# CoderWZW/ARLib

Measured on AMD Instinct MI355X. Metric: BPR-train interactions/sec (LightGCN d=64 L=3 + BPR + Adam, B=2048), higher is better.
Workload: dtype f32

## Files before the change

arlib_amd/_lib.py:

```python
import ctypes as C
import os

_HERE = os.path.dirname(os.path.abspath(__file__))
LIB_PATH = os.environ.get('ARLIB_AMD_LIB') or os.path.join(_HERE, 'lib', 'libarlib_amd.so')
ABI_VERSION = 27
_lib = None


class ArlError(RuntimeError):
    pass


class arl_csr(C.Structure):
    _fields_ = [('n_rows', C.c_int64), ('nnz', C.c_int64), ('rowptr', C.c_void_p), ('col', C.c_void_p), ('val', C.c_void_p),
                ('chunk', C.c_int32), ('n_chunks', C.c_int64), ('chunk_row', C.c_void_p), ('chunk_begin', C.c_void_p),
                ('chunk_end', C.c_void_p), ('n_long', C.c_int64), ('long_row', C.c_void_p), ('long_first', C.c_void_p),
                ('long_count', C.c_void_p), ('partial', C.c_void_p), ('row_tasks', C.c_void_p)]


class arl_blocked(C.Structure):
    _fields_ = [('n_waves', C.c_int64), ('rows_per_wave', C.c_int64), ('loads_in_flight', C.c_int64), ('wave_ptr', C.c_void_p), ('wave_rows', C.c_void_p), ('rec_col', C.c_void_p),
                ('rec_val', C.c_void_p), ('n_split', C.c_int64), ('split_row', C.c_void_p), ('split_first', C.c_void_p), ('split_count', C.c_void_p),
                ('partial', C.c_void_p), ('waves_per_group', C.c_int64)]


class arl_tiled(C.Structure):
    _fields_ = [('n_sweeps', C.c_int64), ('n_slots', C.c_int64), ('cap', C.c_int64), ('n_cb', C.c_int64), ('nnz', C.c_int64),
                ('n_groups', C.c_int64), ('bin_rows', C.c_void_p), ('seg_ptr', C.c_void_p), ('e_col', C.c_void_p), ('e_val', C.c_void_p),
                ('e_row', C.c_void_p)]


_vp, _i64, _i32, _f = C.c_void_p, C.c_int64, C.c_int32, C.c_float
_SIGS = {
    'arl_abi_version': (C.c_int, []),
    'arl_mt_seed': (C.c_int, [_vp, _vp, _i64]),
    'arl_sampler_shuffle': (C.c_int, [_vp, _vp, _i64]),
    'arl_mt_sample_range': (C.c_int, [_vp, _i64, _i64, C.c_int32, _vp, _vp]),
    'arl_sampler_next_batch': (C.c_int, [_vp, _vp, _i64, _i64, _i32, _vp, _vp, _i64, _vp, _vp, _vp]),
    'arl_norm_adj_values_f32': (C.c_int, [_i64, _vp, _vp, _vp, _vp, _vp, _vp]),
    'arl_norm_adj_values_coo_f32': (C.c_int, [_i64, _vp, _vp, _vp, _vp, _i64, _vp, _vp, _vp]),
    'arl_norm_vals_coo_f32': (C.c_int, [_vp, _vp, _vp, _i64, _vp, _vp, _vp]),
    'arl_spmm_csr_f32': (C.c_int, [C.POINTER(arl_csr), _vp, _i64, _f, _f, _vp, _vp, _vp]),
    'arl_spmm_csr_layersum_f32': (C.c_int, [C.POINTER(arl_csr), _vp, _i64, _vp, _vp, _vp, _vp]),
    'arl_spmm_csr_adam_f32': (C.c_int, [C.POINTER(arl_csr), _vp, _i64, _f, _f, _vp, _vp, _vp, _vp, _vp, _f, _f, _f, _f, _i64, _vp]),
    'arl_spmm_blocked_f32': (C.c_int, [C.POINTER(arl_blocked), _vp, _i64, _f, _f, _vp, _vp, _vp, _vp]),
    'arl_spmm_csr_rscale_f32': (C.c_int, [C.POINTER(arl_csr), _vp, _i64, _vp, _f, _f, _vp, _vp, _vp]),
    'arl_spmm_blocked_rscale_f32': (C.c_int, [C.POINTER(arl_blocked), _vp, _i64, _vp, _f, _f, _vp, _vp, _vp]),
    'arl_spmm_blocked_layersum_f32': (C.c_int, [C.POINTER(arl_blocked), _vp, _i64, _vp, _vp, _vp, _vp]),
    'arl_spmm_blocked_adam_f32': (C.c_int, [C.POINTER(arl_blocked), _vp, _i64, _f, _f, _vp, _vp, _vp, _vp, _vp, _f, _f, _f, _f, _i64, _vp]),
    'arl_lpt_deal': (C.c_int, [_i64, _vp, _i64, _i64, _vp, _vp]),
    'arl_syn_v1_pairs': (_i64, [_i64, _i64, C.c_double, C.c_uint64, C.c_double, _i64, _i64, _vp, _i64]),
    'arl_graph_digest': (C.c_uint64, [_vp, _i64]),
    'arl_spmm_tiled_f32': (C.c_int, [C.POINTER(arl_tiled), _vp, _i64, _f, _f, _vp, _vp, _vp, _vp]),
    'arl_spmm_tiled_adam_f32': (C.c_int, [C.POINTER(arl_tiled), _vp, _i64, _f, _f, _vp, _vp, _vp, _vp, _vp, _f, _f, _f, _f, _i64, _vp]),
    'arl_spmm_csr_flagged_f32': (C.c_int, [C.POINTER(arl_csr), _vp, _i64, _vp, _f, _f, _vp, _vp, _vp, _vp]),
    'arl_spmm_csr_rows_workspace_bytes': (_i64, [_i64, _i64, _i64]),
    'arl_spmm_csr_rows_f32': (C.c_int, [C.POINTER(arl_csr), _vp, _i64, _vp, _i64, _i64, _vp, _i64, _f, _vp, _vp, _vp, _vp]),
    'arl_mark_rows_u8': (C.c_int, [_vp, _vp, _i64, _i32, _vp]),
    'arl_mark_rows_bits_u32': (C.c_int, [_vp, _vp, _i64, _i32, _vp]),
    'arl_zero_rows_f32': (C.c_int, [_vp, _vp, _i64, _i64, _vp]),
    'arl_batch_rows_set_f32': (C.c_int, [_vp, _vp, _vp, _vp, _i64, _i64, _vp, _f, _vp, _vp, _vp]),
    'arl_batch_rows_clear_f32': (C.c_int, [_vp, _vp, _vp, _vp, _i64, _i64, _vp, _vp]),
    'arl_bpr_l2_workspace_bytes': (_i64, [_i64]),
    'arl_bpr_l2_fwd_bwd_f32': (C.c_int, [_vp, _i64, _i64, _vp, _vp, _vp, _i64, _f, _f, _vp, _vp, _vp, _i32, _vp]),
    'arl_bpr_l2_partial_f32': (C.c_int, [_vp, _i64, _i64, _vp, _vp, _vp, _i64, _i64, _vp, _vp, _vp]),
    'arl_bpr_l2_backward_f32': (C.c_int, [_vp, _i64, _i64, _vp, _vp, _vp, _i64, _f, _f, _vp, _vp, _vp, _vp]),
    'arl_adam_dense_f32': (C.c_int, [_vp, _vp, _vp, _vp, _i64, _f, _f, _f, _f, _i64, _vp]),
    'arl_sgd_dense_f32': (C.c_int, [_vp, _vp, _i64, _f, _vp]),
    'arl_gather_rows_f32': (C.c_int, [_vp, _vp, _i64, _i64, _vp, _vp]),
    'arl_scatter_add_rows_f32': (C.c_int, [_vp, _vp, _i64, _i64, _vp, _f, _vp]),
    'arl_rows_axpy_unique_f32': (C.c_int, [_vp, _vp, _vp, _i64, _i64, _f, _vp, _vp]),
    'arl_shard_batch_prep_i32': (C.c_int, [_vp, _vp, _vp, _i64, _i64, _i64, _vp, _vp, _vp, _vp, _vp]),
    'arl_infonce_workspace_bytes': (_i64, [_i64, _i64]),
    'arl_infonce_fwd_bwd_f32': (C.c_int, [_vp, _vp, _i64, _i64, _f, _f, _vp, _vp, _vp, _vp, _vp]),
    'arl_simgcl_perturb_f32': (C.c_int, [_vp, _vp, _i64, _i64, _f, _vp]),
    'arl_simgcl_perturb_rng_f32': (C.c_int, [_vp, _vp, _i64, _i64, _vp, _f, C.c_uint64, C.c_uint64, _vp]),
    'arl_ngcf_combine_f32': (C.c_int, [_vp, _vp, _i64, _i64, _vp, _vp]),
    'arl_ngcf_act_f32': (C.c_int, [_vp, _vp, _i64, _i64, _f, _vp]),
    'arl_ngcf_act_bwd_f32': (C.c_int, [_vp, _vp, _i64, _i64, _f, _vp, _vp]),
    'arl_ngcf_combine_bwd_f32': (C.c_int, [_vp, _vp, _vp, _i64, _i64, _vp, _vp, _vp]),
    'arl_ngcf_dense_fwd_f32': (C.c_int, [_vp, _vp, _vp, _i64, _i64, _f, _vp, _vp]),
    'arl_ngcf_dense_dgrad_f32': (C.c_int, [_vp, _vp, _vp, _vp, _vp, _i64, _i64, _f, _vp, _vp, _vp, _vp]),
    'arl_ngcf_wgrad_workspace_bytes': (_i64, [_i64, _i64]),
    'arl_ngcf_dense_wgrad_f32': (C.c_int, [_vp, _vp, _vp, _i64, _i64, _vp, _vp, _vp]),
    'arl_ncf_tower_fwd_f32': (C.c_int, [_vp, _vp, _vp, _i64, _i64, _vp, _vp, _vp, _vp, _vp, _vp, _vp, _vp, _vp, _vp]),
    'arl_ncf_tower_bwd_workspace_bytes': (_i64, [_i64, _i64]),
    'arl_ncf_tower_bwd_f32': (C.c_int, [_vp, _vp, _vp, _vp, _vp, _vp, _i64, _i64, _vp, _vp, _vp, _vp, _vp, _vp, _vp]),
    'arl_wrmf_l2_workspace_bytes': (_i64, [_i64]),
    'arl_wrmf_l2_fwd_bwd_f32': (C.c_int, [_vp, _i64, _i64, _vp, _vp, _vp, _i64, _f, _f, _f, _vp, _vp, _vp, _i32, _vp]),
    'arl_sfa_workspace_bytes': (_i64, [_i64, _i64]),
    'arl_sfa_l1_fwd_bwd_f32': (C.c_int, [_vp, _vp, _vp, _i64, _i64, _i64, _f, C.c_int32, _vp, _vp, _vp, _vp]),
    'arl_sfa_stage1_f32': (C.c_int, [_vp, _vp, _vp, _i64, _i64, _vp, _vp, _vp]),
    'arl_sfa_stage2_f32': (C.c_int, [_vp, _vp, _vp, _i64, _i64, _vp, _vp, _vp]),
    'arl_sfa_stage3_f32': (C.c_int, [_vp, _vp, _vp, _vp, _vp, _i64, _i64, _i64, _f, C.c_int32, _vp, _vp, _vp, _vp]),
    'arl_sddmm_csr_f32': (C.c_int, [_vp, _vp, _i64, _i64, _vp, _vp, _f, _vp, _vp]),
    'arl_sddmm_rows_dense_f32': (C.c_int, [_vp, _vp, _i64, _vp, _i64, _i64, _i64, _vp, _vp]),
    'arl_pga_update_f32': (C.c_int, [_vp, _vp, _vp, _vp, _i64, _i64, _vp]),
    'arl_tables_sum_f32': (C.c_int, [_vp, _i64, _i64, C.c_float, _vp, _vp]),
    'arl_fake_block_rows_workspace_bytes': (_i64, [_i64, _i64, _i64]),
    'arl_fake_block_rows_f32': (C.c_int, [_vp, _i64, _i64, _vp, _i64, _vp, C.c_float, _vp, _vp, _vp]),
    'arl_fake_block_cols_f32': (C.c_int, [_vp, _i64, _i64, _vp, _i64, _vp, C.c_float, _vp, _vp]),
    'arl_cw_topk_term_workspace_bytes': (_i64, [_i64, _i64, _i64, _i64]),
    'arl_cw_topk_term_f32': (C.c_int, [_vp, _i64, _i64, _i64, _i64, _vp, _i64, _vp, _i64, C.c_float, _vp, _vp, _vp, _vp, _vp]),
    'arl_score_mask_topk_workspace_bytes': (_i64, [_i64, _i64]),
    'arl_score_mask_topk_stats_offset': (_i64, [_i64, _i64]),
    'arl_score_mask_topk_user_workspace_bytes': (_i64, [_i64, _i64]),
    'arl_score_mask_topk_f32': (C.c_int, [_vp, _vp, _i64, _i64, _i64, _vp, _vp, _i64, _vp, _vp, _vp, _vp, _vp, _vp, C.c_int32, _vp, _vp]),
    'arl_normalize_rows_f32': (C.c_int, [_vp, _i64, _i64, _vp, _vp, _vp]),
    'arl_normalize_rows_bwd_f32': (C.c_int, [_vp, _vp, _vp, _i64, _i64, _f, _vp, _vp, _vp]),
    'arl_nce_allrows_workspace_bytes': (_i64, [_i64, _i64, _i64]),
    'arl_nce_allrows_lse_f32': (C.c_int, [_vp, _i64, _vp, _i64, _i64, _f, _vp, _vp, _vp]),
    'arl_nce_allrows_grad_f32': (C.c_int, [_vp, _i64, _vp, _i64, _i64, _f, _vp, C.c_int32, _vp, _vp, _vp, _vp]),
    'arl_ssl_dropout_nce_workspace_bytes': (_i64, [_i64, _i64]),
    'arl_ssl_dropout_nce_f32': (C.c_int, [_vp, _vp, _i64, _i64, _f, _f, _f, C.c_uint64, C.c_uint64, _vp, _vp, _vp, _vp, _vp, _vp]),
    'arl_gan_gemm_f32': (C.c_int, [_i64, _i64, _i64, _vp, _i64, _i64, _vp, _i64, _i64, _vp, _i32, _vp, _vp, _vp]),
    'arl_gan_spmm_f32': (C.c_int, [_i64, _i64, _vp, _vp, _vp, _vp, _vp, _i32, _vp, _vp]),
    'arl_gan_transpose_f32': (C.c_int, [_vp, _i64, _i64, _vp, _vp]),
    'arl_gan_rows_f32': (C.c_int, [_vp, _vp, _i64, _i64, _i64, _vp, _vp, _vp, _vp, _vp, _vp, _vp]),
    'arl_gan_dz2_f32': (C.c_int, [_vp, _vp, _vp, _vp, _vp, _i64, _i64, _i64, _vp, _vp]),
    'arl_gan_colsum_workspace_bytes': (_i64, [_i64, _i64]),
    'arl_gan_colsum_f32': (C.c_int, [_vp, _vp, _vp, _vp, _i64, _i64, _vp, _vp, _vp]),
    'arl_gan_hash_key': (C.c_uint64, [C.c_uint64, C.c_uint64]),
    'arl_gan_template_i32': (C.c_int, [_i64, _i64, _i64, _vp, _vp, _vp, _vp, _vp, _vp, _vp, _vp, C.c_uint64, C.c_uint64, _vp, _vp, _vp, _vp, _vp]),
    'arl_gan_hash_mask_u8': (C.c_int, [_i64, _i64, _vp, _vp, C.c_uint64, C.c_uint64, _vp, _vp]),
    'arl_gan_threshold_f32': (C.c_int, [_vp, _i64, _i64, _f, _vp, _vp, _vp, _vp]),
    'arl_comm_load': (C.c_int, [C.c_char_p]),
    'arl_comm_unique_id': (C.c_int, [_vp]),
    'arl_comm_init': (C.c_int, [_vp, _i64, _i64, _i64, C.POINTER(C.c_void_p)]),
    'arl_comm_destroy': (C.c_int, [_vp]),
    'arl_item_exchange_range': (C.c_int, [_i64, _i64, _i64, _i64, _i64, C.POINTER(_i64), C.POINTER(_i64)]),
    'arl_allreduce_item_workspace_bytes': (_i64, [_i64, _i64, _i64]),
    'arl_allreduce_item_f32': (C.c_int, [_vp, _vp, _i64, _i64, _vp, _vp]),
    'arl_topn_project_rows_f32': (C.c_int, [_vp, _i64, _i64, _i64, _vp, _vp, _vp, _vp]),
}
EXPORTS = tuple(_SIGS)


def lib():
    global _lib
    if _lib is None:
        if not os.path.exists(LIB_PATH):
            raise ArlError('arlib_amd: %s is missing -- the HIP extension is the product and there is no CPU fallback. '
                           'Build it with `make -C arlib_amd/csrc` (hipcc --offload-arch=gfx950).' % LIB_PATH)
        import torch
        l = C.CDLL(LIB_PATH)
        for name, (res, args) in _SIGS.items():
            fn = getattr(l, name)
            fn.restype, fn.argtypes = res, args
        if l.arl_abi_version() != ABI_VERSION:
            raise ArlError('arlib_amd: ABI version mismatch (lib %d, python %d): rebuild' % (l.arl_abi_version(), ABI_VERSION))
        _lib = l
    return _lib


_ERR = {-1: 'ARL_E_NULL (required pointer is NULL)', -2: 'ARL_E_DIM (unsupported embedding size/shape)',
        -3: 'ARL_E_RANGE (size outside the int32 index range)', -4: 'ARL_E_ARG (inconsistent arguments)'}


def check(rc, what):
    if rc != 0:
        raise ArlError('%s failed: %s' % (what, _ERR.get(rc, 'hipError_t %d' % rc)))
```

arlib_amd/csrc/arl_host.cpp:

```cpp
#include <cstdint>
#include <cstddef>
#include <queue>
#include <cmath>
#include <algorithm>
#include <utility>
#include <vector>
#include "arlib_amd.h"

namespace {

class PyMersenne {
public:
    explicit PyMersenne(uint32_t *state) : w_(state), pos_(state[kN]) {}
    ~PyMersenne() { w_[kN] = pos_; }

    uint32_t next32() {
        if (pos_ >= kN) refill();
        uint32_t y = w_[pos_++];
        y ^= y >> 11;
        y ^= (y << 7) & 0x9d2c5680u;
        y ^= (y << 15) & 0xefc60000u;
        return y ^ (y >> 18);
    }

    uint32_t below(uint32_t n) {
        if (n == 0) return 0;
        const int shift = __builtin_clz(n);
        uint32_t r;
        do { r = next32() >> shift; } while (r >= n);
        return r;
    }

    static void seed_by_array(uint32_t *w, const uint32_t *key, int64_t len) {
        w[0] = 19650218u;
        for (uint32_t i = 1; i < kN; ++i) w[i] = 1812433253u * (w[i - 1] ^ (w[i - 1] >> 30)) + i;
        uint32_t i = 1;
        int64_t j = 0;
        for (int64_t k = (len > (int64_t)kN ? len : (int64_t)kN); k > 0; --k) {
            w[i] = (w[i] ^ ((w[i - 1] ^ (w[i - 1] >> 30)) * 1664525u)) + key[j] + (uint32_t)j;
            if (++i >= kN) { w[0] = w[kN - 1]; i = 1; }
            if (++j >= len) j = 0;
        }
        for (uint32_t k = kN - 1; k > 0; --k) {
            w[i] = (w[i] ^ ((w[i - 1] ^ (w[i - 1] >> 30)) * 1566083941u)) - i;
            if (++i >= kN) { w[0] = w[kN - 1]; i = 1; }
        }
        w[0] = 0x80000000u;
        w[kN] = kN;
    }

private:
    static constexpr uint32_t kN = 624, kM = 397;
    static uint32_t twist(uint32_t hi, uint32_t lo, uint32_t far) {
        const uint32_t y = (hi & 0x80000000u) | (lo & 0x7fffffffu);
        return far ^ (y >> 1) ^ ((y & 1u) ? 0x9908b0dfu : 0u);
    }
    void refill() {
        for (uint32_t k = 0; k < kN - kM; ++k) w_[k] = twist(w_[k], w_[k + 1], w_[k + kM]);
        for (uint32_t k = kN - kM; k < kN - 1; ++k) w_[k] = twist(w_[k], w_[k + 1], w_[k + kM - kN]);
        w_[kN - 1] = twist(w_[kN - 1], w_[0], w_[kM - 1]);
        pos_ = 0;
    }
    uint32_t *w_;
    uint32_t pos_;
};

inline bool user_has_item(const int64_t *rowptr, const int32_t *items, int64_t rows, int32_t user, int32_t item) {
    if (user < 0 || user >= rows) return false;
    const int32_t *lo = items + rowptr[user], *hi = items + rowptr[user + 1];
    while (lo < hi) {
        const int32_t *mid = lo + (hi - lo) / 2;
        if (*mid < item) lo = mid + 1; else hi = mid;
    }
    return lo < items + rowptr[user + 1] && *lo == item;
}

}

extern "C" {

int arl_abi_version(void) { return 27; }

int arl_mt_seed(uint32_t *mt_state, const uint32_t *key, int64_t key_len) {
    if (!mt_state || !key) return ARL_E_NULL;
    if (key_len < 1) return ARL_E_ARG;
    PyMersenne::seed_by_array(mt_state, key, key_len);
    return ARL_OK;
}

int arl_sampler_shuffle(uint32_t *mt_state, int32_t *pairs, int64_t nnz) {
    if (!mt_state || (!pairs && nnz > 0)) return ARL_E_NULL;
    if (nnz < 0 || nnz > 0xFFFFFFFFll) return ARL_E_RANGE;
    if (mt_state[624] > 624) return ARL_E_ARG;
    PyMersenne rng(mt_state);
    int64_t *rows = reinterpret_cast<int64_t *>(pairs);
    const bool aligned = (reinterpret_cast<uintptr_t>(pairs) & 7u) == 0;
    constexpr int kAhead = 512;
    int64_t js[kAhead];
    for (int64_t i = nnz - 1; i >= 1;) {
        const int cnt = (int)(i < kAhead ? i : kAhead);
        for (int t = 0; t < cnt; ++t) {
            js[t] = rng.below((uint32_t)(i - t + 1));
            __builtin_prefetch(pairs + 2 * js[t], 1, 0);
        }
        if (aligned) {
            for (int t = 0; t < cnt; ++t) { const int64_t a = i - t, j = js[t], v = rows[a]; rows[a] = rows[j]; rows[j] = v; }
        } else {
            for (int t = 0; t < cnt; ++t)
                for (int c = 0; c < 2; ++c) { const int64_t a = i - t, j = js[t]; const int32_t v = pairs[2 * a + c]; pairs[2 * a + c] = pairs[2 * j + c]; pairs[2 * j + c] = v; }
        }
        i -= cnt;
    }
    return ARL_OK;
}

int arl_mt_sample_range(uint32_t *mt_state, int64_t n, int64_t k, int32_t use_pool, int32_t *out, int32_t *scratch) {
    if (!mt_state || (!out && k > 0) || !scratch) return ARL_E_NULL;
    if (n < 0 || k < 0 || k > n || n > 0x7FFFFFFFll) return ARL_E_ARG;
    if (mt_state[624] > 624) return ARL_E_ARG;
    PyMersenne rng(mt_state);
    if (use_pool) {
        for (int64_t i = 0; i < n; ++i) scratch[i] = (int32_t)i;
        for (int64_t i = 0; i < k; ++i) {
            const uint32_t j = rng.below((uint32_t)(n - i));
            out[i] = scratch[j];
            scratch[j] = scratch[n - i - 1];
        }
    } else {
        uint32_t *seen = reinterpret_cast<uint32_t *>(scratch);
        for (int64_t w = 0; w < (n + 31) / 32; ++w) seen[w] = 0u;
        for (int64_t i = 0; i < k; ++i) {
            uint32_t j = rng.below((uint32_t)n);
            while ((seen[j >> 5] >> (j & 31)) & 1u) j = rng.below((uint32_t)n);
            seen[j >> 5] |= 1u << (j & 31);
            out[i] = (int32_t)j;
        }
    }
    return ARL_OK;
}

int arl_sampler_next_batch(uint32_t *mt_state, const int32_t *pairs, int64_t begin, int64_t count, int32_t n_items,
                           const int64_t *memb_rowptr, const int32_t *memb_items, int64_t memb_rows,
                           int32_t *out_u, int32_t *out_p, int32_t *out_n) {
    if (!mt_state || !pairs || !out_u || !out_p || !out_n) return ARL_E_NULL;
    if (memb_rows > 0 && (!memb_rowptr || !memb_items)) return ARL_E_NULL;
    if (begin < 0 || count < 0 || n_items <= 0) return ARL_E_ARG;
    if (mt_state[624] > 624) return ARL_E_ARG;
    PyMersenne rng(mt_state);
    for (int64_t b = 0; b < count; ++b) {
        const int32_t user = pairs[2 * (begin + b)], pos = pairs[2 * (begin + b) + 1];
        int32_t neg;
        do { neg = (int32_t)rng.below((uint32_t)n_items); }
        while (user_has_item(memb_rowptr, memb_items, memb_rows, user, neg));
        out_u[b] = user; out_p[b] = pos; out_n[b] = neg;
    }
    return ARL_OK;
}

int arl_lpt_deal(int64_t n, const int32_t *weight_desc, int64_t n_bins, int64_t cap, int32_t *bin_out, int32_t *slot_out) {
    if (n < 0 || n_bins < 0 || cap < 1 || n_bins > 0x7fffffffll || n_bins * cap < n) return ARL_E_ARG;
    if (n == 0) return ARL_OK;
    if (!weight_desc || !bin_out || !slot_out) return ARL_E_NULL;
    typedef std::pair<int64_t, int32_t> Load;
    std::priority_queue<Load, std::vector<Load>, std::greater<Load>> open;
    std::vector<int32_t> fill((size_t)n_bins, 0);
    for (int64_t b = 0; b < n_bins; ++b) open.push(Load(0, (int32_t)b));
    for (int64_t r = 0; r < n; ++r) {
        if (weight_desc[r] < 0 || (r > 0 && weight_desc[r] > weight_desc[r - 1])) return ARL_E_ARG;
        const Load top = open.top();
        open.pop();
        bin_out[r] = top.second;
        slot_out[r] = fill[top.second]++;
        if (fill[top.second] < cap) open.push(Load(top.first + weight_desc[r], top.second));
    }
    return ARL_OK;
}

static inline uint64_t syn_splitmix64(uint64_t x) {
    x += 0x9E3779B97F4A7C15ull;
    uint64_t z = x;
    z = (z ^ (z >> 30)) * 0xBF58476D1CE4E5B9ull;
    z = (z ^ (z >> 27)) * 0x94D049BB133111EBull;
    return z ^ (z >> 31);
}
static inline uint64_t syn_hash(uint64_t base, uint64_t index) { return syn_splitmix64(index ^ base); }
static inline uint64_t syn_base(uint64_t seed, uint64_t stream) { return syn_splitmix64(seed ^ (stream * 0x9E3779B97F4A7C15ull)); }
static inline double syn_uniform(uint64_t h) { return ((double)(h >> 11) + 0.5) * (1.0 / 9007199254740992.0); }

int64_t arl_syn_v1_pairs(int64_t n_users, int64_t n_items, double mean_deg, uint64_t seed, double sigma, int64_t deg_min, int64_t deg_max,
                         int32_t *pairs_out, int64_t capacity) {
    if (n_users <= 0 || n_items <= 0 || n_users > 0x7fffffffll || n_items > 0x7fffffffll || !(mean_deg > 0) || !(sigma >= 0) || deg_min < 0 || deg_max < deg_min)
        return ARL_E_ARG;
    const uint64_t b1 = syn_base(seed, 1), b2 = syn_base(seed, 2), b3 = syn_base(seed, 3), b4 = syn_base(seed, 4), b5 = syn_base(seed, 5);
    const double mu = std::log(mean_deg) - 0.5 * sigma * sigma;
    const double two_pi = 2.0 * 3.14159265358979323846;
    const int64_t hi = deg_max < n_items ? deg_max : n_items;
    std::vector<int64_t> deg((size_t)n_users);
    int64_t total = 0;
    for (int64_t u = 0; u < n_users; ++u) {
        const double u1 = syn_uniform(syn_hash(b1, (uint64_t)u)), u2 = syn_uniform(syn_hash(b2, (uint64_t)u));
        const double z = std::sqrt(-2.0 * std::log(u1)) * std::cos(two_pi * u2);
        double dg = std::nearbyint(std::exp(mu + sigma * z));
        if (dg < (double)deg_min) dg = (double)deg_min;
        if (dg > (double)hi) dg = (double)hi;
        deg[(size_t)u] = (int64_t)dg;
        total += deg[(size_t)u];
    }
    std::vector<std::pair<uint64_t, int64_t>> hp((size_t)n_items);
    for (int64_t j = 0; j < n_items; ++j) hp[(size_t)j] = std::make_pair(syn_hash(b4, (uint64_t)j), j);
    std::stable_sort(hp.begin(), hp.end(), [](const std::pair<uint64_t, int64_t> &a, const std::pair<uint64_t, int64_t> &b) { return a.first < b.first; });
    std::vector<int64_t> keys;
    keys.reserve((size_t)(total + n_items));
    int64_t k = 0;
    for (int64_t u = 0; u < n_users; ++u)
        for (int64_t t = 0; t < deg[(size_t)u]; ++t, ++k) {
            const double r = syn_uniform(syn_hash(b3, (uint64_t)k));
            int64_t pos = (int64_t)((double)n_items * r * r);
            if (pos > n_items - 1) pos = n_items - 1;
            keys.push_back(u * n_items + hp[(size_t)pos].second);
        }
    for (int64_t j = 0; j < n_items; ++j) keys.push_back((int64_t)(syn_hash(b5, (uint64_t)j) % (uint64_t)n_users) * n_items + j);
    std::sort(keys.begin(), keys.end());
    keys.erase(std::unique(keys.begin(), keys.end()), keys.end());
    const int64_t nnz = (int64_t)keys.size();
    if (!pairs_out || capacity < nnz) return nnz;
    for (int64_t e = 0; e < nnz; ++e) {
        pairs_out[2 * e] = (int32_t)(keys[(size_t)e] / n_items);
        pairs_out[2 * e + 1] = (int32_t)(keys[(size_t)e] % n_items);
    }
    return nnz;
}

uint64_t arl_graph_digest(const int32_t *pairs, int64_t n) {
    uint64_t acc = 0;
// ... 10 lines not shown
```

arlib_amd/csrc/arl_kernels.hip:

```cpp
#include <hip/hip_runtime.h>
#include <stdint.h>
#include <math.h>
#include <stdio.h>
#include <stdlib.h>
#include "arlib_amd.h"
#include <type_traits>

#define ARL_LAUNCH_CHECK()                                  \
    do {                                                    \
        hipError_t e__ = hipGetLastError();                 \
        if (e__ != hipSuccess) return (int)e__;             \
    } while (0)

namespace {

constexpr int kWave = 64;
constexpr int kBlock = 256;
constexpr int kWavesPerBlock = kBlock / kWave;

__device__ __forceinline__ float wave_sum(float v) {
#pragma unroll
    for (int off = 32; off > 0; off >>= 1) v += __shfl_xor(v, off);
    return v;
}
// ... 97 lines not shown
            y.x = fmaf(ep.beta, z.x, y.x); y.y = fmaf(ep.beta, z.y, y.y); y.z = fmaf(ep.beta, z.z, y.z); y.w = fmaf(ep.beta, z.w, y.w);
        }
        *reinterpret_cast<float4 *>(ep.Y + o) = y;
    } else if (MODE == EPI_LAYERSUM) {
        const float4 s = *reinterpret_cast<const float4 *>(ep.S_in + o);
        if (ep.Y) *reinterpret_cast<float4 *>(ep.Y + o) = a;
        *reinterpret_cast<float4 *>(ep.S + o) = add4(s, a);
    } else {
        float g[4] = {ep.alpha * a.x, ep.alpha * a.y, ep.alpha * a.z, ep.alpha * a.w};
        if (ep.Z && (!ep.zflags || ep.zflags[row])) {
            const float4 z = *reinterpret_cast<const float4 *>(ep.Z + o);
            g[0] = fmaf(ep.beta, z.x, g[0]); g[1] = fmaf(ep.beta, z.y, g[1]); g[2] = fmaf(ep.beta, z.z, g[2]); g[3] = fmaf(ep.beta, z.w, g[3]);
        }
        float4 p4 = *reinterpret_cast<const float4 *>(ep.P + o);
        float4 m4 = *reinterpret_cast<const float4 *>(ep.M + o);
        float4 v4 = *reinterpret_cast<const float4 *>(ep.V + o);
        float p[4] = {p4.x, p4.y, p4.z, p4.w}, m[4] = {m4.x, m4.y, m4.z, m4.w}, v[4] = {v4.x, v4.y, v4.z, v4.w};
#pragma unroll
        for (int k = 0; k < 4; ++k) {
            m[k] = m[k] + (g[k] - m[k]) * ep.w1;
            v[k] = v[k] * ep.b2 + ep.w2 * g[k] * g[k];
            const float denom = sqrtf(v[k]) / ep.bc2_sqrt + ep.eps;
            p[k] = p[k] - ep.step_size * (m[k] / denom);
        }
        *reinterpret_cast<float4 *>(ep.P + o) = make_float4(p[0], p[1], p[2], p[3]);
        *reinterpret_cast<float4 *>(ep.M + o) = make_float4(m[0], m[1], m[2], m[3]);
        *reinterpret_cast<float4 *>(ep.V + o) = make_float4(v[0], v[1], v[2], v[3]);
    }
}

template <int LPR, int MODE>
__global__ __launch_bounds__(kBlock) void spmm_rows_kernel(CsrDev A, const float *__restrict__ X, int d, Epi ep) {
    const int lane = threadIdx.x & (kWave - 1);
    const long long task = (long long)blockIdx.x * kWavesPerBlock + (threadIdx.x >> 6);
    const int q = lane % LPR;
    if (task < A.n_chunks) {
        const int t = (int)task;
        float4 a = spmm_gather<LPR, 4>(A.col, A.val, A.chunk_begin[t], A.chunk_end[t], X, d, lane);
        a = group_reduce<LPR>(a);
        if (lane < LPR && q * 4 < d) *reinterpret_cast<float4 *>(A.partial + (size_t)t * d + q * 4) = a;
        return;
    }
    const long long r = task - A.n_chunks;
    if (r >= A.n_rows) return;
    const int begin = A.rowptr[r], end = A.rowptr[r + 1];
    if (A.n_chunks > 0 && end - begin > A.chunk) return;
    float4 a = spmm_gather<LPR, 4>(A.col, A.val, begin, end, X, d, lane);
    a = group_reduce<LPR>(a);
    if (lane < LPR && q * 4 < d) spmm_epilogue<MODE>(ep, (int)r, d, q, a);
}

template <int LPR, int MODE>
__global__ __launch_bounds__(kBlock) void spmm_long_rows_kernel(CsrDev A, int d, Epi ep) {
    constexpr int G = kWave / LPR;
    const int lane = threadIdx.x & (kWave - 1);
    const int t = blockIdx.x * kWavesPerBlock + (threadIdx.x >> 6);
    if (t >= A.n_long) return;
    const int g = lane / LPR, q = lane % LPR;
    const int first = A.long_first[t], cnt = A.long_count[t];
    float4 a = make_float4(0.f, 0.f, 0.f, 0.f);
    if (q * 4 < d)
        for (int s = g; s < cnt; s += G) a = add4(a, *reinterpret_cast<const float4 *>(A.partial + (size_t)(first + s) * d + q * 4));
    a = group_reduce<LPR>(a);
    if (lane < LPR && q * 4 < d) spmm_epilogue<MODE>(ep, A.long_row[t], ep.ld ? ep.ld : d, q, a);
}


template <int LPR, int MODE>
__global__ __launch_bounds__(kBlock) void spmm_rows_masked_gpr_kernel(CsrDev A, const float *__restrict__ X, int d, Epi ep,
                                                                        const uint32_t *__restrict__ xbits) {
    constexpr int G = kWave / LPR;
    const int lane = threadIdx.x & (kWave - 1);
    const int g = lane / LPR, q = lane % LPR;
    const long long task = ((long long)blockIdx.x * kWavesPerBlock + (threadIdx.x >> 6)) * G + g;
    const long long total = (long long)A.n_chunks + A.n_rows;
    int begin = 0, end = 0, row = -1, slot = -1;
    if (task < A.n_chunks) {
        slot = (int)task; begin = A.chunk_begin[slot]; end = A.chunk_end[slot];
    } else if (task < total) {
        if (A.row_tasks) {
            const int4 rt = A.row_tasks[task - A.n_chunks];
            row = rt.x; begin = rt.y; end = rt.z;
        } else {
            row = (int)(task - A.n_chunks);
            begin = A.rowptr[row]; end = A.rowptr[row + 1];
        }
        if (A.n_chunks > 0 && end - begin > A.chunk) { end = begin; row = -1; }
    }
    const bool qact = (q * 4 < d);
    const float *xq = X + q * 4;
    float4 acc = make_float4(0.f, 0.f, 0.f, 0.f);
    for (int base = begin; __any(base < end); base += 2 * LPR) {
        const int e0 = base + q, e1 = base + LPR + q;
        int c0 = 0, c1 = 0;
        if (e0 < end) c0 = A.col[e0];
        if (e1 < end) c1 = A.col[e1];
        bool f0 = false, f1 = false;
        if (e0 < end) f0 = (xbits[c0 >> 5] >> (c0 & 31)) & 1u;
        if (e1 < end) f1 = (xbits[c1 >> 5] >> (c1 & 31)) & 1u;
        const unsigned long long wm0 = __ballot(f0), wm1 = __ballot(f1);
#pragma unroll
        for (int half = 0; half < 2; ++half) {
            const unsigned long long wm = half ? wm1 : wm0;
            const int c = half ? c1 : c0;
            unsigned long long mask = (wm >> (g * LPR)) & ((LPR == 64) ? ~0ull : ((1ull << (LPR & 63)) - 1ull));
            while (mask) {
                const int j = __ffsll((long long)mask) - 1;
                mask &= mask - 1ull;
                const int cj = __shfl(c, g * LPR + j);
                const float vj = A.val[base + half * LPR + j];
                if (qact) fma4(acc, vj, *reinterpret_cast<const float4 *>(xq + (size_t)cj * d));
            }
        }
    }
    if (!qact) return;
    if (slot >= 0) *reinterpret_cast<float4 *>(A.partial + (size_t)slot * d + q * 4) = acc;
    else if (row >= 0) spmm_epilogue<MODE>(ep, row, d, q, acc);
}

struct LayerPtrs { const float *p[8]; int n; };

template <int LPR>
__global__ __launch_bounds__(kBlock) void spmm_subset_kernel(CsrDev A, const float *__restrict__ X, int d, const int32_t *__restrict__ rows, int n,
                                                              int nsplit, float *__restrict__ partial) {
    const int lane = threadIdx.x & (kWave - 1);
    const long long task = (long long)blockIdx.x * kWavesPerBlock + (threadIdx.x >> 6);
    if (task >= (long long)n * nsplit) return;
    const int t = (int)(task / nsplit), sp = (int)(task % nsplit);
    const int r = rows[t];
    const int begin = A.rowptr[r], end = A.rowptr[r + 1];
    const int per = (end - begin + nsplit - 1) / nsplit;
    const int b = begin + sp * per, e = min(end, b + per);
    const int q = lane % LPR;
    float4 a = make_float4(0.f, 0.f, 0.f, 0.f);
    if (b < e) a = spmm_gather<LPR, 4>(A.col, A.val, b, e, X, d, lane);
    a = group_reduce<LPR>(a);
    if (lane < LPR && q * 4 < d) *reinterpret_cast<float4 *>(partial + (size_t)task * d + q * 4) = a;
}

template <int LPR>
__global__ __launch_bounds__(kBlock) void subset_finish_kernel(const float *__restrict__ partial, int n, int nsplit, int d, const int32_t *__restrict__ rows,
                                                                LayerPtrs L, float alpha, float *__restrict__ out_c, const float *__restrict__ row_weight) {
    constexpr int G = kWave / LPR;
    const int lane = threadIdx.x & (kWave - 1);
    const int g = lane / LPR, q = lane % LPR;
    const int t = (blockIdx.x * kWavesPerBlock + (threadIdx.x >> 6)) * G + g;
    if (t >= n || q * 4 >= d) return;
    const int r = rows[t];
    float4 a = make_float4(0.f, 0.f, 0.f, 0.f);
    for (int k = 0; k < L.n; ++k) a = add4(a, *reinterpret_cast<const float4 *>(L.p[k] + (size_t)r * d + q * 4));
    for (int s = 0; s < nsplit; ++s) a = add4(a, *reinterpret_cast<const float4 *>(partial + ((size_t)t * nsplit + s) * d + q * 4));
    const float w = row_weight ? alpha * row_weight[t] : alpha;
    *reinterpret_cast<float4 *>(out_c + (size_t)t * d + q * 4) = make_float4(w * a.x, w * a.y, w * a.z, w * a.w);
}

__global__ __launch_bounds__(kBlock) void tables_sum_kernel(LayerPtrs L, long long n4, float alpha, float4 *__restrict__ out) {
    for (long long t = (long long)blockIdx.x * kBlock + threadIdx.x; t < n4; t += (long long)gridDim.x * kBlock) {
        float4 a = reinterpret_cast<const float4 *>(L.p[0])[t];
        for (int k = 1; k < L.n; ++k) a = add4(a, reinterpret_cast<const float4 *>(L.p[k])[t]);
        out[t] = make_float4(alpha * a.x, alpha * a.y, alpha * a.z, alpha * a.w);
    }
}

__global__ __launch_bounds__(kBlock) void mark_rows_kernel(uint8_t *__restrict__ flags, const int32_t *__restrict__ idx, int n, int value) {
    const int t = blockIdx.x * kBlock + threadIdx.x;
    if (t < n) flags[idx[t]] = (uint8_t)value;
}
__global__ __launch_bounds__(kBlock) void mark_bits_kernel(uint32_t *__restrict__ bits, const int32_t *__restrict__ idx, int n, int set) {
    const int t = blockIdx.x * kBlock + threadIdx.x;
    if (t >= n) return;
    const int i = idx[t];
    if (set) atomicOr(bits + (i >> 5), 1u << (i & 31));
    else atomicAnd(bits + (i >> 5), ~(1u << (i & 31)));
}
__global__ __launch_bounds__(kBlock) void zero_rows_kernel(float *__restrict__ dst, const int32_t *__restrict__ idx, int n, int d) {
    const int lane = threadIdx.x & 63;
    const int t = blockIdx.x * kWavesPerBlock + (threadIdx.x >> 6);
    if (t >= n) return;
    float *o = dst + (size_t)idx[t] * d;
    for (int k = lane; k < d; k += kWave) o[k] = 0.f;
}

constexpr int kOrderedWindow = 16384;

template <class RowOf, class OnHit>
__device__ __forceinline__ bool ordered_scan(int c0, int c1, int t, long long row, int lane, RowOf rowof, OnHit on_hit) {
    for (int base = c0; base < c1; base += 256) {
        long long v[4];
#pragma unroll
        for (int i = 0; i < 4; ++i) {
            const int j = base + 64 * i + lane;
            v[i] = j < c1 ? (long long)rowof(j) : -1ll;
        }
#pragma unroll
        for (int i = 0; i < 4; ++i) {
            unsigned long long m = __ballot(v[i] == row);
            const int b0 = base + 64 * i;
            if (b0 < t) {
                const int lim = t - b0;
                if (lim >= 64 ? m != 0ull : (m & ((1ull << lim) - 1ull)) != 0ull) return false;
            }
            while (m) {
                const int tt = b0 + __ffsll((long long)m) - 1;
                m &= m - 1ull;
                on_hit(tt);
            }
        }
    }
    return true;
}

template <class OnHit>
__device__ __forceinline__ bool ordered_scan_lds(const int32_t *srows, int c0, int c1, int t, int row, int lane, OnHit on_hit) {
    const int n = c1 - c0, tl = t - c0;
    for (int base = 0; base < n; base += 512) {
        int v[8];
#pragma unroll
        for (int i = 0; i < 8; ++i) {
            const int j = base + 64 * i + lane;
            v[i] = j < n ? srows[j] : -1;
        }
#pragma unroll
        for (int i = 0; i < 8; ++i) {
            unsigned long long m = __ballot(v[i] == row);
            const int b0 = base + 64 * i;
            if (b0 < tl) {
                const int lim = tl - b0;
                if (lim >= 64 ? m != 0ull : (m & ((1ull << lim) - 1ull)) != 0ull) return false;
            }
            while (m) {
                const int tt = c0 + b0 + __ffsll((long long)m) - 1;
                m &= m - 1ull;
                on_hit(tt);
            }
        }
    }
    return true;
}
template <class OnGroup>
__device__ __forceinline__ bool ordered_scan_lds_groups(const int32_t *srows, int c0, int c1, int t, int row, int lane, OnGroup on_group) {
    const int n = c1 - c0, tl = t - c0;
    for (int base = 0; base < n; base += 512) {
        int v[8];
#pragma unroll
        for (int i = 0; i < 8; ++i) {
            const int j = base + 64 * i + lane;
            v[i] = j < n ? srows[j] : -1;
        }
#pragma unroll
        for (int i = 0; i < 8; ++i) {
            const unsigned long long m = __ballot(v[i] == row);
            const int b0 = base + 64 * i;
            if (b0 < tl) {
                const int lim = tl - b0;
                if (lim >= 64 ? m != 0ull : (m & ((1ull << lim) - 1ull)) != 0ull) return false;
            }
            if (m) on_group(m, c0 + b0);
        }
    }
    return true;
}
template <class RowOf>
__device__ __forceinline__ void stage_rows(int32_t *srows, int c0, int c1, RowOf rowof) {
    for (int j = threadIdx.x; j < c1 - c0; j += kBlock) srows[j] = (int32_t)rowof(c0 + j);
    __syncthreads();
}

__global__ __launch_bounds__(kBlock) void rows_mark_dups_kernel(uint32_t *__restrict__ bits, uint32_t *__restrict__ dup, const int32_t *__restrict__ idx, int n,
                                                                 const float *__restrict__ row_scale) {
    const int t = blockIdx.x * kBlock + threadIdx.x;
    if (t >= n) return;
    if (row_scale && row_scale[t] == 0.f) return;
    const int row = idx[t];
    const uint32_t m = 1u << (row & 31);
    if (atomicOr(bits + (row >> 5), m) & m) atomicOr(dup + (row >> 5), m);
}

template <bool MARK>
__global__ __launch_bounds__(kBlock) void rows_add_ordered_kernel(float *__restrict__ dst, uint8_t *__restrict__ flags, uint32_t *__restrict__ bits,
                                                                   const int32_t *__restrict__ idx, int c0, int c1, int d,
                                                                   const float *__restrict__ src, float scale, const float *__restrict__ row_scale,
                                                                   const uint32_t *__restrict__ dup) {
    extern __shared__ int32_t srows[];
    const int lane = threadIdx.x & 63;
    const int t = c0 + blockIdx.x * kWavesPerBlock + (threadIdx.x >> 6);
    const bool valid = t < c1 && !(row_scale && row_scale[t] == 0.f);
    const int row = valid ? idx[t] : 0;
    float *o = dst + (size_t)row * d;
    const bool fast = valid && dup && !((dup[row >> 5] >> (row & 31)) & 1u);
    if (fast) {
        const float sc = row_scale ? scale * row_scale[t] : scale;
        const float *s = src + (size_t)t * d;
        for (int k = lane; k < d; k += kWave) {
#pragma clang fp contract(off)
            const float c = sc * s[k];
            o[k] = o[k] + c;
        }
        if (MARK && lane == 0) flags[row] = 1;
    }
    if (!__syncthreads_or(valid && !fast)) return;
    stage_rows(srows, c0, c1, [&](int j) { return (row_scale && row_scale[j] == 0.f) ? -1 : idx[j]; });
    if (!valid || fast) return;
    for (int k0 = 0; k0 < d; k0 += 256) {
        float acc[4];
#pragma unroll
        for (int i = 0; i < 4; ++i) { const int k = k0 + 64 * i + lane; acc[i] = k < d ? o[k] : 0.f; }
// ... 3633 lines not shown
    if (beta != 0.f && !Z) return ARL_E_NULL;
    if (Y == X) return ARL_E_ARG;
    Epi ep = {};
    ep.alpha = alpha; ep.beta = beta; ep.Z = (beta != 0.f) ? Z : nullptr; ep.Y = Y;
    return launch_spmm<EPI_AXPBY>(A, X, d, ep, (hipStream_t)stream);
}

int arl_spmm_csr_rscale_f32(const arl_csr *A, const float *X, int64_t d, const float *row_scale, float alpha, float beta, const float *Z, float *Y,
                            arl_stream_t stream) {
    if (!Y || !row_scale) return ARL_E_NULL;
    if (beta != 0.f && !Z) return ARL_E_NULL;
    if (Y == X) return ARL_E_ARG;
    Epi ep = {};
    ep.alpha = alpha; ep.beta = beta; ep.Z = (beta != 0.f) ? Z : nullptr; ep.Y = Y; ep.rscale = row_scale;
    return launch_spmm<EPI_AXPBY>(A, X, d, ep, (hipStream_t)stream);
}

int arl_spmm_csr_layersum_f32(const arl_csr *A, const float *X, int64_t d, const float *S_in, float *S, float *Y, arl_stream_t stream) {
    if (!S_in || !S) return ARL_E_NULL;
    if (Y == X) return ARL_E_ARG;
    Epi ep = {};
    ep.S_in = S_in; ep.S = S; ep.Y = Y;
    return launch_spmm<EPI_LAYERSUM>(A, X, d, ep, (hipStream_t)stream);
}

int arl_spmm_blocked_f32(const arl_blocked *P, const float *X, int64_t d, float alpha, float beta, const float *Z, const uint8_t *zflags, float *Y,
                         arl_stream_t stream) {
    if (!Y) return ARL_E_NULL;
    if (beta != 0.f && !Z) return ARL_E_NULL;
    if (Y == X) return ARL_E_ARG;
    Epi ep = {};
    ep.alpha = alpha; ep.beta = beta; ep.Z = (beta != 0.f) ? Z : nullptr; ep.zflags = zflags; ep.Y = Y;
    return launch_spmm_blocked<EPI_AXPBY>(P, X, d, ep, (hipStream_t)stream);
}

int arl_spmm_blocked_rscale_f32(const arl_blocked *P, const float *X, int64_t d, const float *row_scale, float alpha, float beta, const float *Z,
                                float *Y, arl_stream_t stream) {
    if (!Y || !row_scale) return ARL_E_NULL;
    if (beta != 0.f && !Z) return ARL_E_NULL;
    if (Y == X) return ARL_E_ARG;
    Epi ep = {};
    ep.alpha = alpha; ep.beta = beta; ep.Z = (beta != 0.f) ? Z : nullptr; ep.Y = Y; ep.rscale = row_scale;
    return launch_spmm_blocked<EPI_AXPBY>(P, X, d, ep, (hipStream_t)stream);
}

int arl_spmm_blocked_layersum_f32(const arl_blocked *P, const float *X, int64_t d, const float *S_in, float *S, float *Y, arl_stream_t stream) {
    if (!S_in || !S) return ARL_E_NULL;
    if (Y == X) return ARL_E_ARG;
    Epi ep = {};
    ep.S_in = S_in; ep.S = S; ep.Y = Y;
    return launch_spmm_blocked<EPI_LAYERSUM>(P, X, d, ep, (hipStream_t)stream);
}

int arl_spmm_blocked_adam_f32(const arl_blocked *P, const float *X, int64_t d, float alpha, float beta, const float *Z, const uint8_t *zflags,
                              float *Pm, float *M, float *V, float lr, float beta1, float beta2, float eps, int64_t step, arl_stream_t stream) {
    if (!Pm || !M || !V) return ARL_E_NULL;
    if (beta != 0.f && !Z) return ARL_E_NULL;
    if (step < 1 || Pm == X) return ARL_E_ARG;
    Epi ep = {};
    ep.alpha = alpha; ep.beta = beta; ep.Z = (beta != 0.f) ? Z : nullptr; ep.zflags = zflags; ep.P = Pm; ep.M = M; ep.V = V;
    {
        const AdamScalars a = adam_scalars(lr, beta1, beta2, step);
        ep.step_size = a.step_size; ep.bc2_sqrt = a.bc2_sqrt; ep.w1 = a.w1; ep.b2 = a.b2; ep.w2 = a.w2; ep.eps = (float)typed_double(eps);
    }
    return launch_spmm_blocked<EPI_ADAM>(P, X, d, ep, (hipStream_t)stream);
}

int arl_spmm_tiled_f32(const arl_tiled *T, const float *X, int64_t d, float alpha, float beta, const float *Z, const uint8_t *zflags, float *Y,
                       arl_stream_t stream) {
    if (!Y) return ARL_E_NULL;
    if (beta != 0.f && !Z) return ARL_E_NULL;
    if (Y == X) return ARL_E_ARG;
    Epi ep = {};
    ep.alpha = alpha; ep.beta = beta; ep.Z = (beta != 0.f) ? Z : nullptr; ep.zflags = zflags; ep.Y = Y;
    return launch_spmm_tiled<EPI_AXPBY>(T, X, d, ep, (hipStream_t)stream);
}

int arl_spmm_tiled_adam_f32(const arl_tiled *T, const float *X, int64_t d, float alpha, float beta, const float *Z, const uint8_t *zflags,
                            float *P, float *M, float *V, float lr, float beta1, float beta2, float eps, int64_t step, arl_stream_t stream) {
    if (!P || !M || !V) return ARL_E_NULL;
    if (beta != 0.f && !Z) return ARL_E_NULL;
    if (step < 1 || P == X) return ARL_E_ARG;
    Epi ep = {};
    ep.alpha = alpha; ep.beta = beta; ep.Z = (beta != 0.f) ? Z : nullptr; ep.zflags = zflags; ep.P = P; ep.M = M; ep.V = V;
    {
        const AdamScalars a = adam_scalars(lr, beta1, beta2, step);
        ep.step_size = a.step_size; ep.bc2_sqrt = a.bc2_sqrt; ep.w1 = a.w1; ep.b2 = a.b2; ep.w2 = a.w2; ep.eps = (float)typed_double(eps);
    }
    return launch_spmm_tiled<EPI_ADAM>(T, X, d, ep, (hipStream_t)stream);
}

int arl_spmm_csr_flagged_f32(const arl_csr *A, const float *X, int64_t d, const uint32_t *xbits, float alpha, float beta, const float *Z,
                             const uint8_t *zflags, float *Y, arl_stream_t stream) {
    if (!Y) return ARL_E_NULL;
    if (beta != 0.f && !Z) return ARL_E_NULL;
    if (Y == X) return ARL_E_ARG;
    Epi ep = {};
    ep.alpha = alpha; ep.beta = beta; ep.Z = (beta != 0.f) ? Z : nullptr; ep.zflags = zflags; ep.Y = Y;
    return launch_spmm<EPI_AXPBY>(A, X, d, ep, (hipStream_t)stream, xbits);
}

int arl_spmm_csr_adam_f32(const arl_csr *A, const float *X, int64_t d, float alpha, float beta, const float *Z, const uint8_t *zflags, float *P,
                          float *M, float *V, float lr, float beta1, float beta2, float eps, int64_t step, arl_stream_t stream) {
    if (!P || !M || !V) return ARL_E_NULL;
    if (beta != 0.f && !Z) return ARL_E_NULL;
    if (step < 1) return ARL_E_ARG;
    if (P == X) return ARL_E_ARG;
    Epi ep = {};
    ep.alpha = alpha; ep.beta = beta; ep.Z = (beta != 0.f) ? Z : nullptr; ep.zflags = zflags; ep.P = P; ep.M = M; ep.V = V;
    {
        const AdamScalars a = adam_scalars(lr, beta1, beta2, step);
        ep.step_size = a.step_size; ep.bc2_sqrt = a.bc2_sqrt; ep.w1 = a.w1; ep.b2 = a.b2; ep.w2 = a.w2; ep.eps = (float)typed_double(eps);
    }
    return launch_spmm<EPI_ADAM>(A, X, d, ep, (hipStream_t)stream);
}

int64_t arl_spmm_csr_rows_workspace_bytes(int64_t n_rows_sel, int64_t nsplit, int64_t d) {
    return (n_rows_sel < 0 || nsplit < 1 || d < 0) ? 0 : (int64_t)sizeof(float) * n_rows_sel * nsplit * d;
}

int arl_spmm_csr_rows_f32(const arl_csr *A, const float *X, int64_t d, const int32_t *rows, int64_t n_rows_sel, int64_t nsplit,
                          const float *const *layers, int64_t n_layers, float alpha, const float *row_weight, float *out_c, void *workspace,
                          arl_stream_t stream) {
    if (!A || !X || !rows || !out_c || !workspace || !A->rowptr) return ARL_E_NULL;
    if (A->nnz > 0 && (!A->col || !A->val)) return ARL_E_NULL;
    if (n_layers < 0 || n_layers > 8 || (n_layers > 0 && !layers)) return ARL_E_ARG;
    if (d <= 0 || d > 256 || (d & 3)) return ARL_E_DIM;
    if (n_rows_sel < 0 || nsplit < 1 || nsplit > 1024 || n_rows_sel * nsplit > 0x7fffffffll) return ARL_E_RANGE;
    if (n_rows_sel == 0) return ARL_OK;
    hipStream_t st = (hipStream_t)stream;
    CsrDev D = {};
    D.n_rows = (int)A->n_rows; D.rowptr = A->rowptr; D.col = A->col; D.val = A->val;
    LayerPtrs LP = {};
    LP.n = (int)n_layers;
    for (int k = 0; k < LP.n; ++k) { if (!layers[k]) return ARL_E_NULL; LP.p[k] = layers[k]; }
    const long long tasks = n_rows_sel * nsplit;
    const unsigned grid = (unsigned)((tasks + kWavesPerBlock - 1) / kWavesPerBlock);
    const int di = (int)d, n = (int)n_rows_sel, ns = (int)nsplit;
    float *part = (float *)workspace;
#define ARL_SUBSET_CASE(LPRV)                                                                                                  \
    do {                                                                                                                       \
        hipLaunchKernelGGL((spmm_subset_kernel<LPRV>), dim3(grid), dim3(kBlock), 0, st, D, X, di, rows, n, ns, part);          \
        ARL_LAUNCH_CHECK();                                                                                                    \
        const unsigned g2 = (unsigned)((n + kWavesPerBlock * (kWave / LPRV) - 1) / (kWavesPerBlock * (kWave / LPRV)));         \
        hipLaunchKernelGGL((subset_finish_kernel<LPRV>), dim3(g2), dim3(kBlock), 0, st, part, n, ns, di, rows, LP, alpha, out_c, row_weight); \
        ARL_LAUNCH_CHECK();                                                                                                    \
    } while (0)
    if (d <= 16) ARL_SUBSET_CASE(4);
    else if (d <= 32) ARL_SUBSET_CASE(8);
    else if (d <= 64) ARL_SUBSET_CASE(16);
    else if (d <= 128) ARL_SUBSET_CASE(32);
    else ARL_SUBSET_CASE(64);
#undef ARL_SUBSET_CASE
    return ARL_OK;
}

int arl_mark_rows_u8(uint8_t *flags, const int32_t *idx, int64_t n, int32_t value, arl_stream_t stream) {
    if (!flags || !idx) return ARL_E_NULL;
    if (n < 0 || n > 0x7fffffffll) return ARL_E_ARG;
    if (n == 0) return ARL_OK;
    hipLaunchKernelGGL(mark_rows_kernel, dim3((unsigned)((n + kBlock - 1) / kBlock)), dim3(kBlock), 0, (hipStream_t)stream, flags, idx, (int)n, (int)value);
    ARL_LAUNCH_CHECK();
    return ARL_OK;
}

int arl_mark_rows_bits_u32(uint32_t *bits, const int32_t *idx, int64_t n, int32_t set, arl_stream_t stream) {
    if (!bits || !idx) return ARL_E_NULL;
    if (n < 0 || n > 0x7fffffffll) return ARL_E_ARG;
    if (n == 0) return ARL_OK;
    hipLaunchKernelGGL(mark_bits_kernel, dim3((unsigned)((n + kBlock - 1) / kBlock)), dim3(kBlock), 0, (hipStream_t)stream, bits, idx, (int)n, (int)set);
    ARL_LAUNCH_CHECK();
    return ARL_OK;
}

int arl_batch_rows_set_f32(float *G, uint8_t *flags, uint32_t *bits, const int32_t *idx, int64_t n, int64_t d, const float *src, float scale,
                           const float *row_scale, uint32_t *dup_bits, arl_stream_t stream) {
    if (!G || !flags || !bits || !idx || !src) return ARL_E_NULL;
    if (n < 0 || n > 0x7fffffffll || d <= 0 || d > 0x7fffffffll) return ARL_E_ARG;
    if (n == 0) return ARL_OK;
    if (dup_bits) {
        hipLaunchKernelGGL(rows_mark_dups_kernel, dim3((unsigned)((n + kBlock - 1) / kBlock)), dim3(kBlock), 0, (hipStream_t)stream, bits, dup_bits, idx, (int)n, row_scale);
        ARL_LAUNCH_CHECK();
    }
    for (int64_t c0 = 0; c0 < n; c0 += kOrderedWindow) {
        const int64_t c1 = c0 + kOrderedWindow < n ? c0 + kOrderedWindow : n;
        hipLaunchKernelGGL(rows_add_ordered_kernel<true>, dim3((unsigned)((c1 - c0 + kWavesPerBlock - 1) / kWavesPerBlock)), dim3(kBlock), (size_t)(c1 - c0) * 4,
                           (hipStream_t)stream, G, flags, bits, idx, (int)c0, (int)c1, (int)d, src, scale, row_scale, (const uint32_t *)dup_bits);
        ARL_LAUNCH_CHECK();
    }
    return ARL_OK;
}

int arl_batch_rows_clear_f32(float *G, uint8_t *flags, uint32_t *bits, const int32_t *idx, int64_t n, int64_t d, uint32_t *dup_bits, arl_stream_t stream) {
    if (!G || !flags || !bits || !idx) return ARL_E_NULL;
    if (n < 0 || n > 0x7fffffffll || d <= 0 || d > 0x7fffffffll) return ARL_E_ARG;
    if (n == 0) return ARL_OK;
    hipLaunchKernelGGL(batch_rows_clear_kernel, dim3((unsigned)((n + kWavesPerBlock - 1) / kWavesPerBlock)), dim3(kBlock), 0, (hipStream_t)stream, G, flags,
                       bits, idx, (int)n, (int)d, dup_bits);
    ARL_LAUNCH_CHECK();
    return ARL_OK;
}

int arl_zero_rows_f32(float *dst, const int32_t *idx, int64_t n, int64_t d, arl_stream_t stream) {
    if (!dst || !idx) return ARL_E_NULL;
    if (n < 0 || d <= 0 || n > 0x7fffffffll || d > 0x7fffffffll) return ARL_E_ARG;
    if (n == 0) return ARL_OK;
    hipLaunchKernelGGL(zero_rows_kernel, dim3((unsigned)((n + kWavesPerBlock - 1) / kWavesPerBlock)), dim3(kBlock), 0, (hipStream_t)stream, dst, idx, (int)n, (int)d);
    ARL_LAUNCH_CHECK();
    return ARL_OK;
}

int64_t arl_bpr_l2_workspace_bytes(int64_t B) { return B < 0 ? 0 : (int64_t)sizeof(float) * 4 * B; }

int arl_bpr_l2_fwd_bwd_f32(const float *emb, int64_t d, int64_t item_off, const int32_t *u, const int32_t *p, const int32_t *n, int64_t B,
                           float reg, float upstream, float *loss_out, float *G, void *workspace, int32_t distinct_rows, arl_stream_t stream) {
    if (!emb || !u || !p || !n || !loss_out || !workspace) return ARL_E_NULL;
    if (d <= 0 || B <= 0 || item_off < 0) return ARL_E_ARG;
    if (B > 0x7fffffffll / 4 || d > 0x7fffffffll) return ARL_E_RANGE;
    hipStream_t st = (hipStream_t)stream;
    float *ws = (float *)workspace;
    const unsigned grid = (unsigned)((B + kWavesPerBlock - 1) / kWavesPerBlock);
    hipLaunchKernelGGL(bpr_fwd_kernel, dim3(grid), dim3(kBlock), 0, st, emb, (int)d, (long long)item_off, u, p, n, (int)B, (float)B, ws);
    ARL_LAUNCH_CHECK();
    hipLaunchKernelGGL(bpr_finalize_kernel, dim3(1), dim3(kBlock), 0, st, (int)B, reg, ws, loss_out, 0);
    ARL_LAUNCH_CHECK();
    if (G) {
        const int rc = launch_bpr_bwd(emb, d, item_off, u, p, n, B, reg, upstream, ws, loss_out, G, st, distinct_rows != 0);
        if (rc) return rc;
    }
    return ARL_OK;
}

int arl_bpr_l2_partial_f32(const float *emb, int64_t d, int64_t item_off, const int32_t *u, const int32_t *p, const int32_t *n, int64_t B_local,
                           int64_t B_global, float *sums_out, void *workspace, arl_stream_t stream) {
    if (!emb || !sums_out || !workspace) return ARL_E_NULL;
    if (B_local > 0 && (!u || !p || !n)) return ARL_E_NULL;
    if (d <= 0 || B_local < 0 || B_global < B_local || B_global <= 0 || item_off < 0) return ARL_E_ARG;
    if (B_local > 0x7fffffffll / 4 || d > 0x7fffffffll) return ARL_E_RANGE;
    hipStream_t st = (hipStream_t)stream;
    float *ws = (float *)workspace;
    if (B_local > 0) {
        const unsigned grid = (unsigned)((B_local + kWavesPerBlock - 1) / kWavesPerBlock);
        hipLaunchKernelGGL(bpr_fwd_kernel, dim3(grid), dim3(kBlock), 0, st, emb, (int)d, (long long)item_off, u, p, n, (int)B_local, (float)B_global, ws);
        ARL_LAUNCH_CHECK();
    }
    hipLaunchKernelGGL(bpr_finalize_kernel, dim3(1), dim3(kBlock), 0, st, (int)B_local, 0.f, ws, sums_out, 1);
    ARL_LAUNCH_CHECK();
    return ARL_OK;
}

int arl_bpr_l2_backward_f32(const float *emb, int64_t d, int64_t item_off, const int32_t *u, const int32_t *p, const int32_t *n, int64_t B_local,
                            float reg, float upstream, const float *norms4, float *G, const void *workspace, arl_stream_t stream) {
    if (!emb || !norms4 || !G || !workspace) return ARL_E_NULL;
    if (B_local > 0 && (!u || !p || !n)) return ARL_E_NULL;
    if (d <= 0 || B_local < 0 || item_off < 0) return ARL_E_ARG;
    if (B_local > 0x7fffffffll / 4 || d > 0x7fffffffll) return ARL_E_RANGE;
    if (B_local == 0) return ARL_OK;
    return launch_bpr_bwd(emb, d, item_off, u, p, n, B_local, reg, upstream, (const float *)workspace, norms4, G, (hipStream_t)stream);
}

int arl_adam_dense_f32(float *p, const float *g, float *m, float *v, int64_t n, float lr, float beta1, float beta2, float eps, int64_t step,
                       arl_stream_t stream) {
    if (!p || !g || !m || !v) return ARL_E_NULL;
    if (n < 0 || step < 1) return ARL_E_ARG;
    if (n == 0) return ARL_OK;
    const AdamScalars a = adam_scalars(lr, beta1, beta2, step);
    hipStream_t st = (hipStream_t)stream;
    const bool al = (((uintptr_t)p | (uintptr_t)g | (uintptr_t)m | (uintptr_t)v) & 15u) == 0;
    const long long n4 = al ? n / 4 : 0;
    if (n4 > 0) {
        hipLaunchKernelGGL(adam_kernel, dim3(grid_for(n4, kBlock)), dim3(kBlock), 0, st, (float4 *)p, (const float4 *)g, (float4 *)m, (float4 *)v, n4,
                           a.step_size, a.bc2_sqrt, a.w1, a.b2, a.w2, eps);
        ARL_LAUNCH_CHECK();
    }
    if (n4 * 4 < n) {
        hipLaunchKernelGGL(adam_scalar_kernel, dim3(grid_for(n - n4 * 4, kBlock)), dim3(kBlock), 0, st, p, g, m, v, n4 * 4, (long long)n, a.step_size,
                           a.bc2_sqrt, a.w1, a.b2, a.w2, eps);
        ARL_LAUNCH_CHECK();
    }
    return ARL_OK;
}

int arl_sgd_dense_f32(float *p, const float *g, int64_t n, float lr, arl_stream_t stream) {
    if (!p || !g) return ARL_E_NULL;
    if (n < 0) return ARL_E_ARG;
    if (n == 0) return ARL_OK;
    hipLaunchKernelGGL(sgd_kernel, dim3(grid_for(n, kBlock)), dim3(kBlock), 0, (hipStream_t)stream, p, g, (long long)n, lr);
    ARL_LAUNCH_CHECK();
    return ARL_OK;
}

int arl_tables_sum_f32(const float *const *tables, int64_t n_tables, int64_t n_elems, float alpha, float *out, arl_stream_t stream) {
    if (!tables || !out) return ARL_E_NULL;
    if (n_tables < 1 || n_tables > 8 || n_elems < 0 || (n_elems & 3)) return ARL_E_ARG;
    if (n_elems == 0) return ARL_OK;
    LayerPtrs LP = {};
    LP.n = (int)n_tables;
    for (int k = 0; k < LP.n; ++k) { if (!tables[k]) return ARL_E_NULL; LP.p[k] = tables[k]; }
    const long long n4 = n_elems / 4;
    hipLaunchKernelGGL(tables_sum_kernel, dim3(grid_for(n4, kBlock)), dim3(kBlock), 0, (hipStream_t)stream, LP, n4, alpha, (float4 *)out);
    ARL_LAUNCH_CHECK();
    return ARL_OK;
}

int arl_gather_rows_f32(const float *src, const int32_t *idx, int64_t n, int64_t d, float *dst, arl_stream_t stream) {
    if (!src || !idx || !dst) return ARL_E_NULL;
// ... 912 lines not shown
```

arlib_amd/engine.py:

```python
import torch

from . import ops


def mean_adjacency_gradient(A, E0, G, L, s, out, noises=None, eps=0.1):
    if L == 0:
        return out
    E = [E0]
    for k in range(L - 1):
        nxt = ops.spmm(A, E[-1])
        if noises is not None:
            ops.simgcl_perturb_(nxt, noises[k], eps)
        E.append(nxt)
    G = G.contiguous()
    acc = G
    for j in range(L):
        ops.sddmm_csr(A, acc, E[L - 1 - j], s, out=out)
        if j < L - 1:
            acc = ops.spmm(A, acc, 1.0, 1.0, G)
    return out


class PropagationEngine:
    def __init__(self, graph, n_users, n_items, emb_size, n_layers, reg, lr, device, skip_layer0=False,
                 optimizer='adam', betas=(0.9, 0.999), eps=1e-8, table=None, schedule='auto'):
        self.A = graph
        self.U, self.I, self.d, self.L = int(n_users), int(n_items), int(emb_size), int(n_layers)
        self.N = self.U + self.I
        self.reg, self.lr, self.betas, self.eps = float(reg), float(lr), betas, eps
        self.skip0 = bool(skip_layer0)
        self.optimizer = optimizer
        self.device = torch.device(device)
        if self.device.type != 'cuda':
            raise ops._lib.ArlError('PropagationEngine needs a GPU device (no CPU fallback)')
        if graph is None and self.L > 0:
            raise ValueError('n_layers > 0 needs a graph')
        if graph is not None and graph.n_rows != self.N:
            raise ValueError('graph has %d rows, expected U+I=%d' % (graph.n_rows, self.N))
        if self.L > 0:
            ops._check_width(self.d, 'PropagationEngine')
        if self.skip0 and self.L < 1:
            raise ValueError('skip_layer0 needs n_layers >= 1')
        if schedule not in ('auto', 'csr', 'blocked'):
            raise ValueError("schedule must be 'auto', 'csr' or 'blocked'")
        if schedule != 'csr':
            ops.auto_blocked(graph, emb_size, split=self.U, force=(schedule == 'blocked'))
        if graph is not None and graph.nnz >= ops.BLOCKED_MIN_NNZ:
            graph.enable_masked_order()
        z = lambda: torch.zeros(self.N, self.d, dtype=torch.float32, device=self.device)
        self.E0 = z() if table is None else table
        if self.E0.shape != (self.N, self.d) or self.E0.dtype != torch.float32 or not self.E0.is_contiguous():
            raise ValueError('table must be contiguous fp32 [U+I, d]')
        self.m, self.v, self.G = z(), z(), z()
        if self.L > 0:
            self.S, self.Ea, self.Eb = z(), z(), z()
        else:
            self.S = self.E0
        self.t = 0
        self.loss_out = torch.zeros(4, dtype=torch.float32, device=self.device)
        self._G_dirty = True
        self._noise_seed, self._noise_stream = None, 0
        self.nsplit = 32
        self.flags = self.bits = self.dup_bits = self.hops = None
        self._sparse_B, self._sb_cache = None, {}
        self.Gc = self.out_c = self.rows_ws = self.ar = self.arB = self._ws = None
        self._sgl_acc = self._sgl_hops = None
        self.ngcf_W = self.ngcf_m = self.ngcf_v = None

    @property
    def user_emb(self):
        return self.E0[:self.U]

    @property
    def item_emb(self):
        return self.E0[self.U:]

    def forward(self, noises=None, eps=0.1, out=None):
        L, A = self.L, self.A
        if L == 0:
            return self.E0
        S = self.S if out is None else out
        if noises is None and not self.skip0:
            if L == 1:
                return ops.spmm(A, self.E0, 0.5, 0.5, self.E0, out=S)
            ops.spmm_layersum(A, self.E0, self.E0, S, self.Ea)
            cur, nxt = self.Ea, self.Eb
            for _ in range(L - 2):
                ops.spmm_layersum(A, cur, S, S, nxt)
                cur, nxt = nxt, cur
            s = 1.0 / (L + 1)
            return ops.spmm(A, cur, s, s, S, out=S)
        cur, nxt, x = self.Ea, self.Eb, self.E0
        for k in range(L):
            ops.spmm(A, x, out=cur)
            if noises is not None:
                ops.simgcl_perturb_(cur, noises[k], eps)
            if k == 0:
                if self.skip0:
                    S.copy_(cur)
                else:
                    torch.add(self.E0, cur, out=S)
            else:
                S.add_(cur)
            x, cur, nxt = cur, nxt, cur
        S.mul_(1.0 / (L if self.skip0 else L + 1))
        return S

    def backward_to_table(self, G, out=None):
        L, A = self.L, self.A
        if L == 0:
            return G
        acc, dst = self._dense_hops(G)
        if self.skip0:
            return ops.spmm(A, acc, 1.0 / L, out=dst)
        s = 1.0 / (L + 1)
        return ops.spmm(A, acc, s, s, G, out=dst)

    def _dense_hops(self, G):
        acc, bufs = G, (self.Ea, self.Eb)
        for k in range(self.L - 1):
            acc = ops.spmm(self.A, acc, 1.0, 1.0, G, out=bufs[k % 2])
        return acc, bufs[(self.L - 1) % 2]

    def adjacency_gradient(self, G, out=None, noises=None, eps=0.1):
        L, A = self.L, self.A
        if out is None:
            out = torch.zeros(A.col.numel(), dtype=torch.float32, device=G.device)
        return mean_adjacency_gradient(A, self.E0, G, L, 1.0 / L if self.skip0 else 1.0 / (L + 1), out, noises, eps)

    def forward_rows(self, rows):
        L, A = self.L, self.A
        if L == 0 or self.skip0 or L > 8:
            raise ValueError('forward_rows: LightGCN mean over layers 0..L with 1 <= L <= 8')
        n = rows.numel()
        self._sparse_buffers(max(n // 3, 1) if n % 3 == 0 else n)
        return self._mean_rows(A, self.hops, rows)

    def backward_rows(self, rows, g_rows):
        L, A = self.L, self.A
        s = 1.0 / (L + 1)
        self._begin_sparse(self._sparse_B)
        self._set_rows(rows, g_rows.contiguous())
        acc, bits = self._masked_hops(A, self.hops)
        out = ops.spmm_flagged(A, acc, bits, s, s, self.G, self.flags)
        self._clear_rows(rows)
        return out

    def _begin_sparse(self, B):
        self._sparse_buffers(B)
        if self._G_dirty:
            self.G.zero_()
            self._G_dirty = False

    def _batch_rows(self, u, p, n):
        return torch.cat([u, p + self.U, n + self.U])

    def _contrast_rows(self, u, p):
        uidx = torch.unique(u.long())
        iidx = torch.unique(p.long()) + self.U
        return torch.cat([uidx, iidx]).to(torch.int32), uidx.numel()

    def _streams(self, n):
        if self._noise_seed is None:
            self._noise_seed = int(torch.randint(0, 2 ** 62, (1,)).item())
            self._noise_stream = 0
        first = self._noise_stream
        self._noise_stream += n
        return self._noise_seed, first

    def _mean_rows(self, graph, hops, rows, out=None, workspace=None):
        layers = [self.E0]
        for k in range(self.L - 1):
            layers.append(ops.spmm(graph, layers[-1], out=hops[k]))
        return ops.spmm_rows(graph, layers[-1], rows, layers, 1.0 / (self.L + 1), nsplit=self.nsplit, out=out, workspace=workspace, check_range=False)

    def _bpr_compact(self, out_c, B):
        self.Gc.zero_()
        ops.bpr_l2_fwd_bwd(out_c, B, self.ar, self.ar, self.arB, self.reg, self.Gc, workspace=self._ws, loss_out=self.loss_out, check_range=False, distinct_rows=True)

    def _set_rows(self, rows, grad):
        ops.batch_rows_set_(self.G, self.flags, self.bits, rows, grad, 1.0, check_range=False, dup_bits=self.dup_bits)

    def _mark_rows(self, rows):
        ops.mark_rows_(self.flags, rows, 1, check_range=False)
        ops.mark_bits_(self.bits, rows, True, self.N, check_range=False)

    def _clear_rows(self, rows):
        ops.batch_rows_clear_(self.G, self.flags, self.bits, rows, check_range=False, dup_bits=self.dup_bits)

    def _masked_hops(self, graph, bufs, src=None, after_hop=None):
        acc, bits = self.G if src is None else src, self.bits
        for k in range(self.L - 1):
            acc = ops.spmm_flagged(graph, acc, bits, 1.0, 1.0, self.G, self.flags, out=bufs[k % len(bufs)])
            bits = None
            if after_hop is not None:
                after_hop(self.L - 1 - k, acc)
        return acc, bits

    def loss_and_grad_out(self, out, u, p, n):
        self.G.zero_()
        self._G_dirty = True
        if self._ws is None or self._ws.numel() < 4 * u.numel():
            self._ws = torch.empty(4 * u.numel(), dtype=torch.float32, device=self.device)
        ops.bpr_l2_fwd_bwd(out, self.U, u, p, n, self.reg, self.G, workspace=self._ws, loss_out=self.loss_out, check_range=False)
        return self.loss_out

    def grad(self, u, p, n):
        out = self.forward()
        lo = self.loss_and_grad_out(out, u, p, n)
        return lo, self.backward_to_table(self.G)

    def step(self, u, p, n, rows=None):
        if self.optimizer != 'adam' or self.L == 0 or self.skip0 or self.L > 8:
            return self.step_dense(u, p, n)
        return self._step_sparse(u, p, n, rows, None)

    def _step_sparse(self, u, p, n, rows, extra_grad):
        L, A = self.L, self.A
        B = u.numel()
        if rows is None:
            rows = self._batch_rows(u, p, n)
        self._begin_sparse(B)
        s = 1.0 / (L + 1)
        self._mean_rows(A, self.hops, rows, out=self.out_c, workspace=self.rows_ws)
        self._bpr_compact(self.out_c, B)
        if extra_grad is not None:
            extra_grad()
        self._set_rows(rows, self.Gc)
        self.t += 1
        acc, bits = self._masked_hops(A, self.hops)
        if L == 1:
            ops.spmm_flagged(A, acc, bits, s, s, self.G, self.flags, out=self.hops[0])
            ops.adam_dense(self.E0, self.hops[0], self.m, self.v, self.lr, self.t, self.betas, self.eps)
        else:
            ops.spmm_adam(A, acc, s, s, self.G, self.E0, self.m, self.v, self.lr, self.t, self.betas, self.eps, zflags=self.flags)
        self._clear_rows(rows)
        return self.loss_out

    def step_ssl4rec(self, u, p, n, cl_rate=1.0, tau=0.2, drop=0.2, masks=None, seed=None, stream_id=None):
        L, A = self.L, self.A
        if self.optimizer != 'adam' or self.skip0 or L < 1 or L > 8:
            raise ValueError('step_ssl4rec needs a LightGCN-mean engine (no skip_layer0, 1 <= L <= 8) with Adam')
        B = u.numel()
        if self.d not in ops.SSL_NCE_WIDTHS:
            raise ValueError('step_ssl4rec: embedding size %d unsupported (d in %s)' % (self.d, ops.SSL_NCE_WIDTHS))
        if masks is not None and tuple(masks.shape) != (2, 2, B, self.d):
            raise ValueError('step_ssl4rec: masks [2, 2, B, d]')
        if seed is None:
            seed, stream_id = self._streams(1)
        cl = []
        def contrastive():
            loss, _ = ops.ssl_dropout_nce(self.out_c[:B], self.out_c[B:2 * B], drop, tau, G=(self.Gc[:B], self.Gc[B:2 * B]), upstream=cl_rate,
                                          seed=seed, stream_id=stream_id, masks=masks)
            cl.append(loss)
        self._step_sparse(u, p, n, None, contrastive)
        cl = cl[0]
        return self.loss_out, cl_rate * (cl[1] + cl[0])

    def init_ngcf(self, weights):
        if len(weights) != self.L or any(tuple(w.shape) != (self.d, self.d) for pair in weights for w in pair):
            raise ValueError('init_ngcf: one pair of [d, d] weights per layer')
        self.ngcf_W = [(a.data if hasattr(a, 'data') else a, b.data if hasattr(b, 'data') else b) for a, b in weights]
        z = lambda: torch.zeros(self.d, self.d, dtype=torch.float32, device=self.device)
        self.ngcf_m = [(z(), z()) for _ in weights]
        self.ngcf_v = [(z(), z()) for _ in weights]

    def step_ngcf(self, u, p, n, rows=None, slope=0.01, capture=None):
        L, A, d = self.L, self.A, self.d
        if L < 1 or self.ngcf_W is None or d not in ops.NGCF_DENSE_WIDTHS:
            raise ValueError('step_ngcf: needs n_layers >= 1, init_ngcf() and d in %s' % (ops.NGCF_DENSE_WIDTHS,))
        B = u.numel()
        if rows is None:
            rows = self._batch_rows(u, p, n)
        self._begin_sparse(B)
        s = 1.0 / (L + 1)
        Wcat = [torch.cat([a, b], 0) for a, b in self.ngcf_W]
        egos, Ps = [self.E0], []
        for l in range(L - 1):
            P = ops.spmm(A, egos[-1])
            Ps.append(P)
            egos.append(ops.ngcf_dense_fwd(P, egos[-1], Wcat[l], slope))
        P_r = ops.spmm_rows(A, egos[-1], rows, (), 1.0, nsplit=ops.ROWS_NSPLIT, check_range=False)
        E_r = ops.gather_rows(egos[-1], rows, check_range=False)
        out_r = ops.ngcf_dense_fwd(P_r, E_r, Wcat[L - 1], slope)
        acc = out_r + E_r
        for e in egos[:-1]:
            acc += ops.gather_rows(e, rows, check_range=False)
        acc *= s
        self._bpr_compact(acc, B)
        Gs = self.Gc * s
        self.t += 1
        gP_r, gE_r, gW = ops.ngcf_dense_bwd(Gs, out_r, P_r, E_r, Wcat[L - 1], slope)
        gWs = [None] * L
        gWs[L - 1] = gW
        self._set_rows(rows, gP_r)
        g = ops.spmm_flagged(A, self.G, self.bits)
        self._clear_rows(rows)
        ops.scatter_add_rows(g, rows, gE_r + Gs, 1.0, check_range=False)
        if L == 1:
            if capture is not None:
                capture['table'] = g.clone()
            ops.adam_dense(self.E0, g, self.m, self.v, self.lr, self.t, self.betas, self.eps)
        for l in range(L - 2, -1, -1):
            gP, gE, gWs[l] = ops.ngcf_dense_bwd(g, egos[l + 1], Ps[l], egos[l], Wcat[l], slope)
            ops.scatter_add_rows(gE, rows, Gs, 1.0, check_range=False)
            if l > 0:
                g = ops.spmm(A, gP, 1.0, 1.0, gE)
            elif capture is not None:
                capture['table'] = ops.spmm(A, gP, 1.0, 1.0, gE)
                ops.adam_dense(self.E0, capture['table'], self.m, self.v, self.lr, self.t, self.betas, self.eps)
            else:
                ops.spmm_adam(A, gP, 1.0, 1.0, gE, self.E0, self.m, self.v, self.lr, self.t, self.betas, self.eps)
        if capture is not None:
            capture['W'] = [w.clone() for w in gWs]
        for l in range(L):
            for k in range(2):
                ops.adam_dense(self.ngcf_W[l][k], gWs[l][k * d:(k + 1) * d], self.ngcf_m[l][k], self.ngcf_v[l][k], self.lr, self.t, self.betas, self.eps)
        return self.loss_out

    def step_simgcl(self, u, p, n, cl_rate=0.2, tau=0.2, eps=0.1, noises=None):
        if not self.skip0 or self.optimizer != 'adam':
            raise ValueError('step_simgcl needs a skip_layer0 engine with Adam')
        L, A = self.L, self.A
        B = u.numel()
        self._begin_sparse(B)
        inv = 1.0 / L
        rows = self._batch_rows(u, p, n)
        rows_cl, nu = self._contrast_rows(u, p)
        rng_mode = noises is None
        if rng_mode:
            seed, stream0 = self._streams(2 * L)
        rnd = (lambda v, k: noises[v][k]) if noises is not None else None
        def perturb_full(src, v, k, out=None):
            if rng_mode:
                return ops.simgcl_perturb_rng(src, eps, seed, stream0 + v * L + k, out=out)
            dst = src.clone() if out is None else out.copy_(src)
            return ops.simgcl_perturb_(dst, rnd(v, k), eps)
        def perturb_rows(src, v, k, sel):
            if rng_mode:
                return ops.simgcl_perturb_rng(src, eps, seed, stream0 + v * L + k, out=src, row_ids=sel)
            return ops.simgcl_perturb_(src, rnd(v, k)[sel.long()].contiguous(), eps)
        E1 = ops.spmm(A, self.E0, out=self.hops[0])
        def finish(first, view):
            sel = rows if view is None else rows_cl
            layers, cur = [first], first
            for k in range(1, L - 1):
                nxt = ops.spmm(A, cur)
                if view is not None:
                    perturb_full(nxt, view, k, out=nxt)
                layers.append(nxt); cur = nxt
            if L == 1:
                return ops.gather_rows(first, sel, check_range=False)
            if view is None:
                return ops.spmm_rows(A, cur, sel, layers, inv, nsplit=self.nsplit, check_range=False)
            last = ops.spmm_rows(A, cur, sel, (), 1.0, nsplit=self.nsplit, check_range=False)
            perturb_rows(last, view, L - 1, sel)
            for t in layers:
                last += ops.gather_rows(t, sel, check_range=False)
            return last * inv
        out_c = finish(E1, None)
        self._bpr_compact(out_c, B)
        ops.scatter_add_rows(self.G, rows, self.Gc, 1.0, check_range=False)
        views = []
        for v in (0, 1):
            E1p = perturb_full(E1, v, 0)
            views.append(finish(E1p, v))
        lu, du1, du2 = ops.infonce_fwd_bwd(views[0][:nu].contiguous(), views[1][:nu].contiguous(), tau)
        li, di1, di2 = ops.infonce_fwd_bwd(views[0][nu:].contiguous(), views[1][nu:].contiguous(), tau)
        cl_loss = cl_rate * (lu[0] + li[0])
        gcl = torch.cat([du1 + du2, di1 + di2], 0)
        ops.scatter_add_rows(self.G, rows_cl, gcl, cl_rate, check_range=False)
        allrows = torch.cat([rows, rows_cl])
        self._mark_rows(allrows)
        self.t += 1
        acc, bits = self._masked_hops(A, (self.hops[1], self.hops[0]))
        if L == 1:
            tmp = ops.spmm_flagged(A, acc, bits, inv, 0.0, None, None, out=self.hops[1])
            ops.adam_dense(self.E0, tmp, self.m, self.v, self.lr, self.t, self.betas, self.eps)
        else:
            ops.spmm_adam(A, acc, inv, 0.0, None, self.E0, self.m, self.v, self.lr, self.t, self.betas, self.eps)
        self._clear_rows(allrows)
        return self.loss_out, cl_loss

    def step_xsimgcl(self, u, p, n, cl_rate=0.2, tau=0.1, eps=0.1, layer_cl=1, noises=None):
        if not self.skip0 or self.optimizer != 'adam':
            raise ValueError('step_xsimgcl needs a skip_layer0 engine with Adam')
        L, A = self.L, self.A
        if not (1 <= layer_cl <= L):
            raise ValueError('layer_cl must be in [1, L]')
        B = u.numel()
        self._begin_sparse(B)
        inv = 1.0 / L
        rows = self._batch_rows(u, p, n)
        rows_cl, nu = self._contrast_rows(u, p)
        sel = torch.cat([rows, rows_cl])
        rng_mode = noises is None
        if rng_mode:
            seed, stream0 = self._streams(L)
        layers, cur = [], self.E0
        for k in range(L - 1):
            nxt = ops.spmm(A, cur, out=self.hops[k] if L <= 3 else None)
            if rng_mode:
                ops.simgcl_perturb_rng(nxt, eps, seed, stream0 + k, out=nxt)
            else:
                ops.simgcl_perturb_(nxt, noises[k], eps)
            layers.append(nxt); cur = nxt
        last = ops.spmm_rows(A, cur, sel, (), 1.0, nsplit=self.nsplit, check_range=False)
        if rng_mode:
            ops.simgcl_perturb_rng(last, eps, seed, stream0 + L - 1, out=last, row_ids=sel)
        else:
            ops.simgcl_perturb_(last, noises[L - 1][sel.long()].contiguous(), eps)
        mean_c = last.clone()
        for t in layers:
            mean_c += ops.gather_rows(t, sel, check_range=False)
        mean_c *= inv
        cl_c = last[3 * B:] if layer_cl == L else ops.gather_rows(layers[layer_cl - 1], rows_cl, check_range=False)
        self._bpr_compact(mean_c[:3 * B].contiguous(), B)
        mcl = mean_c[3 * B:]
        lu, du1, du2 = ops.infonce_fwd_bwd(mcl[:nu].contiguous(), cl_c[:nu].contiguous(), tau)
        li, di1, di2 = ops.infonce_fwd_bwd(mcl[nu:].contiguous(), cl_c[nu:].contiguous(), tau)
        cl_loss = cl_rate * (lu[0] + li[0])
        g_mean_cl = torch.cat([du1, di1], 0)
        g_layer = torch.cat([du2, di2], 0) * cl_rate
        ops.scatter_add_rows(self.G, rows, self.Gc, inv, check_range=False)
        ops.scatter_add_rows(self.G, rows_cl, g_mean_cl, cl_rate * inv, check_range=False)
        self._mark_rows(sel)
        self.t += 1
        src = self.G
        if layer_cl == L:
            if L > 1:
                src = self.G.clone()
            ops.scatter_add_rows(src, rows_cl, g_layer, 1.0, check_range=False)
        def inject(level, acc):
            if level == layer_cl:
                ops.scatter_add_rows(acc, rows_cl, g_layer, 1.0, check_range=False)
        bufs = (self.hops[1], self.hops[0])
        acc, bits = self._masked_hops(A, bufs, src, inject)
        if L == 1:
            tmp = ops.spmm_flagged(A, acc, bits, 1.0, 0.0, None, None, out=bufs[0])
            ops.adam_dense(self.E0, tmp, self.m, self.v, self.lr, self.t, self.betas, self.eps)
        else:
            ops.spmm_adam(A, acc, 1.0, 0.0, None, self.E0, self.m, self.v, self.lr, self.t, self.betas, self.eps)
        self._clear_rows(sel)
        return self.loss_out, cl_loss

    def step_sgl(self, u, p, n, view1, view2, cl_rate=0.2, tau=0.2):
        if self.skip0 or self.optimizer != 'adam' or self.L < 1:
            raise ValueError('step_sgl needs a LightGCN-style engine (layers 0..L averaged) with Adam')
        L = self.L
        B = u.numel()
        self._begin_sparse(B)
        s = 1.0 / (L + 1)
        rows = self._batch_rows(u, p, n)
        rows_cl, _ = self._contrast_rows(u, p)
        if self._sgl_acc is None:
            self._sgl_acc = torch.empty_like(self.E0)
            self._sgl_hops = [torch.empty_like(self.E0) for _ in range(max(L - 1, 1))]

        def backward_into(graph, sel, grad_c, accumulate):
            self._set_rows(sel, grad_c)
            acc, bits = self._masked_hops(graph, self._sgl_hops)
            tmp = ops.spmm_flagged(graph, acc, bits, s, s, self.G, self.flags, out=self._sgl_hops[0] if L == 1 else self.hops[0])
            if accumulate:
                self._sgl_acc.add_(tmp)
            else:
                self._sgl_acc.copy_(tmp)
            self._clear_rows(sel)

        out_c = self._mean_rows(self.A, self._sgl_hops, rows)
        self._bpr_compact(out_c, B)
        v1 = self._mean_rows(view1, self._sgl_hops, rows_cl)
        v2 = self._mean_rows(view2, self._sgl_hops, rows_cl)
        lcl, d1, d2 = ops.infonce_fwd_bwd(v1, v2, tau)
        cl_loss = cl_rate * lcl[0]
        backward_into(self.A, rows, self.Gc, False)
        backward_into(view1, rows_cl, d1 * cl_rate, True)
        backward_into(view2, rows_cl, d2 * cl_rate, True)
        self.t += 1
        ops.adam_dense(self.E0, self._sgl_acc, self.m, self.v, self.lr, self.t, self.betas, self.eps)
        return self.loss_out, cl_loss

    def _sparse_buffers(self, B):
        if self._sparse_B == B:
            return
        dev, d = self.device, self.d
        if self.flags is None:
            self.flags = torch.zeros(self.N, dtype=torch.uint8, device=dev)
            self.bits = torch.zeros((self.N + 31) // 32, dtype=torch.int32, device=dev)
            self.dup_bits = torch.zeros_like(self.bits)
            self.hops = [self.Ea, self.Eb] + [torch.empty_like(self.Ea) for _ in range(max(0, self.L - 3))]
        sb = self._sb_cache.get(B)
        if sb is None:
            ar = torch.arange(B, dtype=torch.int32, device=dev)
            sb = (torch.zeros(3 * B, d, dtype=torch.float32, device=dev), torch.empty(3 * B, d, dtype=torch.float32, device=dev),
                  torch.empty(3 * B * self.nsplit * d, dtype=torch.float32, device=dev), ar, ar + B, torch.empty(4 * B, dtype=torch.float32, device=dev))
            if len(self._sb_cache) >= 8:
                del self._sb_cache[next(iter(self._sb_cache))]
            self._sb_cache[B] = sb
        self.Gc, self.out_c, self.rows_ws, self.ar, self.arB, self._ws = sb
        self._sparse_B = B

    def step_dense(self, u, p, n):
        L, A = self.L, self.A
        out = self.forward()
        lo = self.loss_and_grad_out(out, u, p, n)
        self.t += 1
        if self.optimizer == 'adam' and L > 0 and not self.skip0:
            acc, _ = self._dense_hops(self.G)
            s = 1.0 / (L + 1)
            ops.spmm_adam(A, acc, s, s, self.G, self.E0, self.m, self.v, self.lr, self.t, self.betas, self.eps)
            return lo
        g = self.backward_to_table(self.G)
        self.apply_grad(g)
        return lo

    def apply_grad(self, g):
        if self.optimizer == 'adam':
            ops.adam_dense(self.E0, g, self.m, self.v, self.lr, self.t, self.betas, self.eps)
        elif self.optimizer == 'sgd':
            ops.sgd_dense(self.E0, g, self.lr)
        else:
            raise ValueError('unknown optimizer %r' % (self.optimizer,))

    def step_bytes(self, B):
        E, N, d, L = (self.A.nnz if self.A is not None else 0), self.N, self.d, self.L
        return L * (16 * E + 8 * N + 24 * N * d) + 28 * N * d + 24 * B * d
```

arlib_amd/ops.py:

```python
import ctypes as C
import os
import time
import numpy as np
import torch

from . import _lib
from ._lib import arl_csr, check

DEFAULT_CHUNK = 512
EVENT_HOOK = None


_raw_stream = getattr(torch._C, '_cuda_getCurrentRawStream', None)


def _stream():
    if _raw_stream is not None:
        return C.c_void_p(_raw_stream(torch.cuda.current_device()))
    return C.c_void_p(torch.cuda.current_stream().cuda_stream)


def _dev(t, dtype, name, ndim=None):
    if not isinstance(t, torch.Tensor):
        raise TypeError('%s: expected a torch.Tensor' % name)
# ... 512 lines not shown
        bp._bind(g, None)
        return bp


def _check_width(d, name, multiple_of_4=True):
    if d <= 0 or d > 256 or (multiple_of_4 and d % 4):
        raise ValueError('%s: embedding size %d unsupported (%s<= 256)' % (name, d, 'multiple of 4, ' if multiple_of_4 else ''))


def _check_xy(A, X, name='X', rows=None):
    _dev(X, torch.float32, name, 2)
    want = A.n_rows if rows is None else rows
    if X.shape[0] != want:
        raise ValueError('%s: %d rows, expected %d' % (name, X.shape[0], want))
    d = X.shape[1]
    _check_width(d, name)
    if X.device != A.device:
        raise ValueError('%s on %s, graph on %s' % (name, X.device, A.device))
    return d


def spmm(A, X, alpha=1.0, beta=0.0, Z=None, out=None, row_scale=None, rows_from=0):
    d = _check_xy(A, X, 'X', A.n_cols)
    Y = torch.empty(A.n_rows, d, dtype=torch.float32, device=X.device) if out is None else out
    if _check_xy(A, Y, 'out') != d or Y.data_ptr() == X.data_ptr():
        raise ValueError('spmm: out must be [n_rows, d] and must not alias X')
    if beta != 0.0:
        if Z is None or _check_xy(A, Z, 'Z') != d:
            raise ValueError('spmm: Z [n_rows, d] required when beta != 0')
    L, zp, st = _lib.lib(), (_ptr(Z) if beta != 0.0 else None), _stream()
    tok = EVENT_HOOK.begin('axpby') if EVENT_HOOK is not None else None
    if row_scale is not None:
        _dev(row_scale, torch.float32, 'row_scale', 1)
        if row_scale.numel() != A.n_rows:
            raise ValueError('spmm: row_scale needs one entry per output row')
        _spmm_dispatch(A, d, lambda p: check(L.arl_spmm_blocked_rscale_f32(p, _ptr(X), d, _ptr(row_scale), alpha, beta, zp, _ptr(Y), st), 'arl_spmm_blocked_rscale_f32'),
                       lambda p: check(L.arl_spmm_csr_rscale_f32(p, _ptr(X), d, _ptr(row_scale), alpha, beta, zp, _ptr(Y), st), 'arl_spmm_csr_rscale_f32'),
                       rows_from=rows_from)
    else:
        _spmm_dispatch(A, d, lambda p: check(L.arl_spmm_blocked_f32(p, _ptr(X), d, alpha, beta, zp, None, _ptr(Y), st), 'arl_spmm_blocked_f32'),
                       lambda p: check(L.arl_spmm_csr_f32(p, _ptr(X), d, alpha, beta, zp, _ptr(Y), st), 'arl_spmm_csr_f32'), rows_from=rows_from)
    if tok is not None:
        EVENT_HOOK.end(tok)
    return Y


def spmm_layersum(A, X, S_in, S, Y=None):
    d = _check_xy(A, X)
    for t, nm in ((S_in, 'S_in'), (S, 'S')):
        _check_xy(A, t, nm)
        if t.shape != X.shape:
            raise ValueError('spmm_layersum: %s shape mismatch' % nm)
    if Y is not None:
        _check_xy(A, Y, 'Y')
        if Y.shape != X.shape or Y.data_ptr() == X.data_ptr():
            raise ValueError('spmm_layersum: Y must not alias X')
    if S.data_ptr() == X.data_ptr():
        raise ValueError('spmm_layersum: S must not alias X')
    L, st = _lib.lib(), _stream()
    tok = EVENT_HOOK.begin('layersum') if EVENT_HOOK is not None else None
    _spmm_dispatch(A, d, lambda p: check(L.arl_spmm_blocked_layersum_f32(p, _ptr(X), d, _ptr(S_in), _ptr(S), _ptr(Y), st), 'arl_spmm_blocked_layersum_f32'),
                   lambda p: check(L.arl_spmm_csr_layersum_f32(p, _ptr(X), d, _ptr(S_in), _ptr(S), _ptr(Y), st), 'arl_spmm_csr_layersum_f32'))
    if tok is not None:
        EVENT_HOOK.end(tok)
    return S


def _check_flags(t, n, name):
    _dev(t, torch.uint8, name, 1)
    if t.numel() != n:
        raise ValueError('%s: %d flags, expected %d' % (name, t.numel(), n))
    return t


def spmm_adam(A, X, alpha, beta, Z, P, M, V, lr, step, betas=(0.9, 0.999), eps=1e-8, zflags=None):
    d = _check_xy(A, X, 'X', A.n_cols)
    for t, nm in ((P, 'P'), (M, 'M'), (V, 'V')):
        if _check_xy(A, t, nm) != d or t.data_ptr() == X.data_ptr():
            raise ValueError('spmm_adam: %s shape/alias error' % nm)
    if beta != 0.0:
        if Z is None or _check_xy(A, Z, 'Z') != d:
            raise ValueError('spmm_adam: Z shape mismatch')
    if zflags is not None:
        _check_flags(zflags, A.n_rows, 'zflags')
    L, zp, st = _lib.lib(), (_ptr(Z) if beta != 0.0 else None), _stream()
    tok = EVENT_HOOK.begin('adam') if EVENT_HOOK is not None else None
    _spmm_dispatch(A, d, lambda p: check(L.arl_spmm_blocked_adam_f32(p, _ptr(X), d, alpha, beta, zp, _ptr(zflags), _ptr(P), _ptr(M), _ptr(V), lr, betas[0],
                                                                     betas[1], eps, int(step), st), 'arl_spmm_blocked_adam_f32'),
                   lambda p: check(L.arl_spmm_csr_adam_f32(p, _ptr(X), d, alpha, beta, zp, _ptr(zflags), _ptr(P), _ptr(M), _ptr(V), lr, betas[0], betas[1], eps,
                                                           int(step), st), 'arl_spmm_csr_adam_f32'))
    if tok is not None:
        EVENT_HOOK.end(tok)


def spmm_flagged(A, X, xflags=None, alpha=1.0, beta=0.0, Z=None, zflags=None, out=None):
    d = _check_xy(A, X, 'X', A.n_cols)
    Y = torch.empty(A.n_rows, d, dtype=torch.float32, device=X.device) if out is None else out
    if _check_xy(A, Y, 'out') != d or Y.data_ptr() == X.data_ptr():
        raise ValueError('spmm_flagged: out must be [n_rows, d] and must not alias X')
    if beta != 0.0 and (Z is None or _check_xy(A, Z, 'Z') != d):
        raise ValueError('spmm_flagged: Z [n_rows, d] required when beta != 0')
    if xflags is not None:
        _dev(xflags, torch.int32, 'xflags (bitmap)', 1)
        if xflags.numel() != (A.n_cols + 31) // 32:
            raise ValueError('spmm_flagged: bitmap needs ceil(n_cols/32) int32 words')
    if zflags is not None:
        _check_flags(zflags, A.n_rows, 'zflags')
    L, zp, st = _lib.lib(), (_ptr(Z) if beta != 0.0 else None), _stream()
    tok = EVENT_HOOK.begin('masked' if xflags is not None else 'axpby') if EVENT_HOOK is not None else None
    csr = lambda p: check(L.arl_spmm_csr_flagged_f32(p, _ptr(X), d, _ptr(xflags), alpha, beta, zp, _ptr(zflags), _ptr(Y), st), 'arl_spmm_csr_flagged_f32')
    if xflags is not None:
        csr(C.byref(A._struct(d)))
    else:
        _spmm_dispatch(A, d, lambda p: check(L.arl_spmm_blocked_f32(p, _ptr(X), d, alpha, beta, zp, _ptr(zflags), _ptr(Y), st), 'arl_spmm_blocked_f32'), csr)
    if tok is not None:
        EVENT_HOOK.end(tok)
    return Y


ROWS_NSPLIT = 16


def spmm_rows(A, X, rows, layers=(), alpha=1.0, nsplit=ROWS_NSPLIT, out=None, workspace=None, check_range=True, row_weight=None):
    d = _check_xy(A, X, 'X', A.n_cols)
    _dev(rows, torch.int32, 'rows', 1)
    n = rows.numel()
    if check_range and n and (int(rows.min()) < 0 or int(rows.max()) >= A.n_rows):
        raise IndexError('spmm_rows: row index out of range')
    if len(layers) > 8:
        raise ValueError('spmm_rows: at most 8 layer tables')
    for t in layers:
        if _check_xy(A, t, 'layer') != d:
            raise ValueError('spmm_rows: layer table shape mismatch')
    if out is None:
        out = torch.empty(n, d, dtype=torch.float32, device=X.device)
    _dev(out, torch.float32, 'out', 2)
    if out.shape != (n, d):
        raise ValueError('spmm_rows: out must be [len(rows), d]')
    need = _lib.lib().arl_spmm_csr_rows_workspace_bytes(n, nsplit, d) // 4
    if workspace is None or workspace.numel() < need:
        workspace = torch.empty(max(need, 1), dtype=torch.float32, device=X.device)
    arr = (C.c_void_p * max(len(layers), 1))(*[t.data_ptr() for t in layers])
    s = A._struct(d)
    tok = EVENT_HOOK.begin('rows') if EVENT_HOOK is not None else None
    if row_weight is not None and (_dev(row_weight, torch.float32, 'row_weight', 1).numel() != n):
        raise ValueError('spmm_rows: row_weight must have one entry per listed row')
    check(_lib.lib().arl_spmm_csr_rows_f32(C.byref(s), _ptr(X), d, _ptr(rows), n, nsplit, C.cast(arr, C.c_void_p), len(layers), alpha, _ptr(row_weight),
                                           _ptr(out), _ptr(workspace), _stream()), 'arl_spmm_csr_rows_f32')
    if tok is not None:
        EVENT_HOOK.end(tok)
    return out


def mark_rows_(flags, idx, value, check_range=True):
    _dev(flags, torch.uint8, 'flags', 1); _dev(idx, torch.int32, 'idx', 1)
    if check_range and idx.numel() and (int(idx.min()) < 0 or int(idx.max()) >= flags.numel()):
        raise IndexError('mark_rows_: index out of range')
    check(_lib.lib().arl_mark_rows_u8(_ptr(flags), _ptr(idx), idx.numel(), int(value), _stream()), 'arl_mark_rows_u8')
    return flags


def batch_rows_set_(G, flags, bits, idx, src, scale=1.0, check_range=True, row_scale=None, dup_bits=None):
    _dev(G, torch.float32, 'G', 2); _dev(flags, torch.uint8, 'flags', 1); _dev(bits, torch.int32, 'bits', 1); _dev(idx, torch.int32, 'idx', 1)
    _dev(src, torch.float32, 'src', 2)
    N, d = G.shape
    if flags.numel() != N or bits.numel() != (N + 31) // 32 or src.shape != (idx.numel(), d):
        raise ValueError('batch_rows_set_: shape mismatch')
    if check_range and idx.numel() and (int(idx.min()) < 0 or int(idx.max()) >= N):
        raise IndexError('batch_rows_set_: index out of range')
    if row_scale is not None and _dev(row_scale, torch.float32, 'row_scale', 1).numel() != idx.numel():
        raise ValueError('batch_rows_set_: row_scale must have one entry per index')
    if dup_bits is not None and _dev(dup_bits, torch.int32, 'dup_bits', 1).numel() != bits.numel():
        raise ValueError('batch_rows_set_: dup_bits must have the size of bits')
    check(_lib.lib().arl_batch_rows_set_f32(_ptr(G), _ptr(flags), _ptr(bits), _ptr(idx), idx.numel(), d, _ptr(src), scale, _ptr(row_scale), _ptr(dup_bits),
                                            _stream()), 'arl_batch_rows_set_f32')


def batch_rows_clear_(G, flags, bits, idx, check_range=True, dup_bits=None):
    _dev(G, torch.float32, 'G', 2); _dev(flags, torch.uint8, 'flags', 1); _dev(bits, torch.int32, 'bits', 1); _dev(idx, torch.int32, 'idx', 1)
    N, d = G.shape
    if flags.numel() != N or bits.numel() != (N + 31) // 32:
        raise ValueError('batch_rows_clear_: shape mismatch')
    if check_range and idx.numel() and (int(idx.min()) < 0 or int(idx.max()) >= N):
        raise IndexError('batch_rows_clear_: index out of range')
    if dup_bits is not None and _dev(dup_bits, torch.int32, 'dup_bits', 1).numel() != bits.numel():
        raise ValueError('batch_rows_clear_: dup_bits must have the size of bits')
    check(_lib.lib().arl_batch_rows_clear_f32(_ptr(G), _ptr(flags), _ptr(bits), _ptr(idx), idx.numel(), d, _ptr(dup_bits), _stream()), 'arl_batch_rows_clear_f32')

def mark_bits_(bits, idx, set_, n_nodes, check_range=True):
    _dev(bits, torch.int32, 'bits', 1); _dev(idx, torch.int32, 'idx', 1)
    if bits.numel() != (n_nodes + 31) // 32:
        raise ValueError('mark_bits_: bitmap size')
    if check_range and idx.numel() and (int(idx.min()) < 0 or int(idx.max()) >= n_nodes):
        raise IndexError('mark_bits_: index out of range')
    check(_lib.lib().arl_mark_rows_bits_u32(_ptr(bits), _ptr(idx), idx.numel(), 1 if set_ else 0, _stream()), 'arl_mark_rows_bits_u32')
    return bits


def zero_rows_(dst, idx, check_range=True):
    _dev(dst, torch.float32, 'dst', 2); _dev(idx, torch.int32, 'idx', 1)
    if check_range and idx.numel() and (int(idx.min()) < 0 or int(idx.max()) >= dst.shape[0]):
        raise IndexError('zero_rows_: index out of range')
    check(_lib.lib().arl_zero_rows_f32(_ptr(dst), _ptr(idx), idx.numel(), dst.shape[1], _stream()), 'arl_zero_rows_f32')
    return dst


def _check_idx(t, name, hi, B=None):
    _dev(t, torch.int32, name, 1)
    if B is not None and t.numel() != B:
        raise ValueError('%s: length %d != %d' % (name, t.numel(), B))
    return t


def bpr_l2_fwd_bwd(emb, item_off, u, p, n, reg, G=None, upstream=1.0, workspace=None, loss_out=None, check_range=True, distinct_rows=False):
    _dev(emb, torch.float32, 'emb', 2)
    N, d = emb.shape
    B = u.numel()
    for t, nm in ((u, 'u'), (p, 'p'), (n, 'n')):
        _check_idx(t, nm, N, B)
    if B == 0:
        raise ValueError('bpr_l2: empty batch')
    if check_range:
        mx = torch.stack([u.max(), p.max(), n.max(), -u.min(), -p.min(), -n.min()]).tolist()
        if mx[0] >= N or max(mx[1], mx[2]) + item_off >= N or max(mx[3:]) > 0:
            raise IndexError('bpr_l2: batch index out of range')
    if G is not None:
        _dev(G, torch.float32, 'G', 2)
        if G.shape != emb.shape:
            raise ValueError('bpr_l2: G shape mismatch')
    need = _lib.lib().arl_bpr_l2_workspace_bytes(B)
    if workspace is None or workspace.numel() * workspace.element_size() < need:
        workspace = torch.empty(need // 4, dtype=torch.float32, device=emb.device)
    if loss_out is None:
        loss_out = torch.empty(4, dtype=torch.float32, device=emb.device)
    check(_lib.lib().arl_bpr_l2_fwd_bwd_f32(_ptr(emb), d, item_off, _ptr(u), _ptr(p), _ptr(n), B, reg, upstream, _ptr(loss_out), _ptr(G),
                                            _ptr(workspace), 1 if distinct_rows else 0, _stream()), 'arl_bpr_l2_fwd_bwd_f32')
    return loss_out


def adam_dense(p, g, m, v, lr, step, betas=(0.9, 0.999), eps=1e-8):
    for t, nm in ((p, 'p'), (g, 'g'), (m, 'm'), (v, 'v')):
        _dev(t, torch.float32, nm)
        if t.numel() != p.numel():
            raise ValueError('adam_dense: size mismatch on %s' % nm)
    check(_lib.lib().arl_adam_dense_f32(_ptr(p), _ptr(g), _ptr(m), _ptr(v), p.numel(), lr, betas[0], betas[1], eps, int(step), _stream()), 'arl_adam_dense_f32')


def sgd_dense(p, g, lr):
    _dev(p, torch.float32, 'p'); _dev(g, torch.float32, 'g')
    if g.numel() != p.numel():
        raise ValueError('sgd_dense: size mismatch')
    check(_lib.lib().arl_sgd_dense_f32(_ptr(p), _ptr(g), p.numel(), lr, _stream()), 'arl_sgd_dense_f32')


def gather_rows(src, idx, check_range=True):
    _dev(src, torch.float32, 'src', 2); _dev(idx, torch.int32, 'idx', 1)
    if check_range and idx.numel() and (int(idx.min()) < 0 or int(idx.max()) >= src.shape[0]):
        raise IndexError('gather_rows: index out of range')
    dst = torch.empty(idx.numel(), src.shape[1], dtype=torch.float32, device=src.device)
    check(_lib.lib().arl_gather_rows_f32(_ptr(src), _ptr(idx), idx.numel(), src.shape[1], _ptr(dst), _stream()), 'arl_gather_rows_f32')
    return dst


def scatter_add_rows(dst, idx, src, scale=1.0, check_range=True):
    _dev(dst, torch.float32, 'dst', 2); _dev(src, torch.float32, 'src', 2); _dev(idx, torch.int32, 'idx', 1)
    if src.shape != (idx.numel(), dst.shape[1]):
        raise ValueError('scatter_add_rows: shape mismatch')
    if check_range and idx.numel() and (int(idx.min()) < 0 or int(idx.max()) >= dst.shape[0]):
        raise IndexError('scatter_add_rows: index out of range')
    check(_lib.lib().arl_scatter_add_rows_f32(_ptr(dst), _ptr(idx), idx.numel(), dst.shape[1], _ptr(src), scale, _stream()), 'arl_scatter_add_rows_f32')
    return dst


def rows_axpy_unique_(dst, src, idx, alpha=1.0, check_range=True, dup_bits=None):
    _dev(dst, torch.float32, 'dst', 2); _dev(src, torch.float32, 'src', 2); _dev(idx, torch.int32, 'idx', 1)
    if src.shape != dst.shape or src.data_ptr() == dst.data_ptr():
        raise ValueError('rows_axpy_unique_: dst and src must be distinct tables of one shape')
    if check_range and idx.numel() and (int(idx.min()) < 0 or int(idx.max()) >= dst.shape[0]):
        raise IndexError('rows_axpy_unique_: index out of range')
    check(_lib.lib().arl_rows_axpy_unique_f32(_ptr(dst), _ptr(src), _ptr(idx), idx.numel(), dst.shape[1], float(alpha), _ptr(dup_bits), _stream()), 'arl_rows_axpy_unique_f32')
    return dst


def shard_batch_prep(u, p, n, u0, u1, out=None):
    for t, nm in ((u, 'u'), (p, 'p'), (n, 'n')):
        _dev(t, torch.int32, nm, 1)
    B = u.numel()
    if p.numel() != B or n.numel() != B or not (0 <= u0 <= u1):
        raise ValueError('shard_batch_prep: u, p, n must have one length and 0 <= u0 <= u1')
    if out is None:
        out = (torch.empty(B, dtype=torch.int32, device=u.device), torch.empty(3 * B, dtype=torch.float32, device=u.device),
               torch.empty(2 * B, dtype=torch.int32, device=u.device), torch.empty(3 * B, dtype=torch.int32, device=u.device))
    lu, own, item_rows, rows_l = out
    check(_lib.lib().arl_shard_batch_prep_i32(_ptr(u), _ptr(p), _ptr(n), B, int(u0), int(u1), _ptr(lu), _ptr(own), _ptr(item_rows), _ptr(rows_l), _stream()),
          'arl_shard_batch_prep_i32')
    return out


def infonce_fwd_bwd(v1, v2, tau, want_grad=True, upstream=1.0):
    _dev(v1, torch.float32, 'v1', 2); _dev(v2, torch.float32, 'v2', 2)
    if v1.shape != v2.shape:
        raise ValueError('infonce: shape mismatch')
    n, d = v1.shape
    if n == 0 or n > 8192 or d % 4 or d > 256:
        raise ValueError('infonce: unsupported shape %s' % (tuple(v1.shape),))
    ws = torch.empty(_lib.lib().arl_infonce_workspace_bytes(n, d) // 4, dtype=torch.float32, device=v1.device)
# ... 997 lines not shown
```

include/arlib_amd.h:

```cpp
#ifndef ARLIB_AMD_H
#define ARLIB_AMD_H

#include <stdint.h>

#ifdef __cplusplus
extern "C" {
#endif

#define ARL_OK 0
#define ARL_E_NULL (-1)
#define ARL_E_DIM (-2)
#define ARL_E_RANGE (-3)
#define ARL_E_ARG (-4)

typedef void *arl_stream_t;

int arl_abi_version(void);

int arl_mt_seed(uint32_t *mt_state, const uint32_t *key, int64_t key_len);
int arl_sampler_shuffle(uint32_t *mt_state, int32_t *pairs, int64_t nnz);
int arl_mt_sample_range(uint32_t *mt_state, int64_t n, int64_t k, int32_t use_pool, int32_t *out, int32_t *scratch);
int arl_sampler_next_batch(uint32_t *mt_state, const int32_t *pairs, int64_t begin, int64_t count,
                           int32_t n_items, const int64_t *memb_rowptr, const int32_t *memb_items,
                           int64_t memb_rows, int32_t *out_u, int32_t *out_p, int32_t *out_n);

typedef struct arl_csr {
    int64_t n_rows;
    int64_t nnz;
    const int32_t *rowptr;
    const int32_t *col;
    const float *val;
    int32_t chunk;
    int64_t n_chunks;
    const int32_t *chunk_row;
    const int32_t *chunk_begin;
    const int32_t *chunk_end;
    int64_t n_long;
    const int32_t *long_row;
    const int32_t *long_first;
    const int32_t *long_count;
    float *partial;
    const int32_t *row_tasks;
} arl_csr;

int arl_norm_adj_values_f32(int64_t n_rows, const int32_t *rowptr, const int32_t *col, const float *w,
                            float *dinv, float *val, arl_stream_t stream);
int arl_norm_adj_values_coo_f32(int64_t n_rows, const int32_t *rowptr, const int32_t *erow, const int32_t *col,
                                const float *w, int64_t nnz, float *dinv, float *val, arl_stream_t stream);
int arl_norm_vals_coo_f32(const int32_t *erow, const int32_t *col, const float *w, int64_t nnz, const float *dinv, float *val,
                          arl_stream_t stream);

int arl_spmm_csr_f32(const arl_csr *A, const float *X, int64_t d, float alpha, float beta, const float *Z,
                     float *Y, arl_stream_t stream);
int arl_spmm_csr_layersum_f32(const arl_csr *A, const float *X, int64_t d, const float *S_in, float *S,
                              float *Y, arl_stream_t stream);
int arl_spmm_csr_adam_f32(const arl_csr *A, const float *X, int64_t d, float alpha, float beta, const float *Z,
                          const uint8_t *zflags, float *P, float *M, float *V, float lr, float beta1, float beta2,
                          float eps, int64_t step, arl_stream_t stream);

int arl_spmm_csr_flagged_f32(const arl_csr *A, const float *X, int64_t d, const uint32_t *xbits, float alpha, float beta,
                             const float *Z, const uint8_t *zflags, float *Y, arl_stream_t stream);
int64_t arl_spmm_csr_rows_workspace_bytes(int64_t n_rows_sel, int64_t nsplit, int64_t d);
int arl_spmm_csr_rows_f32(const arl_csr *A, const float *X, int64_t d, const int32_t *rows, int64_t n_rows_sel,
                          int64_t nsplit, const float *const *layers, int64_t n_layers, float alpha, const float *row_weight,
                          float *out_c, void *workspace, arl_stream_t stream);
int arl_mark_rows_u8(uint8_t *flags, const int32_t *idx, int64_t n, int32_t value, arl_stream_t stream);
int arl_mark_rows_bits_u32(uint32_t *bits, const int32_t *idx, int64_t n, int32_t set, arl_stream_t stream);
int arl_zero_rows_f32(float *dst, const int32_t *idx, int64_t n, int64_t d, arl_stream_t stream);
int arl_batch_rows_set_f32(float *G, uint8_t *flags, uint32_t *bits, const int32_t *idx, int64_t n, int64_t d,
                           const float *src, float scale, const float *row_scale, uint32_t *dup_bits, arl_stream_t stream);
int arl_batch_rows_clear_f32(float *G, uint8_t *flags, uint32_t *bits, const int32_t *idx, int64_t n, int64_t d,
                             uint32_t *dup_bits, arl_stream_t stream);

typedef struct arl_blocked {
    int64_t n_waves, rows_per_wave;
    int64_t loads_in_flight;
    const int32_t *wave_ptr;
    const int32_t *wave_rows;
    const int32_t *rec_col;
    const float *rec_val;
    int64_t n_split;
    const int32_t *split_row;
    const int32_t *split_first;
    const int32_t *split_count;
    float *partial;
    int64_t waves_per_group;
} arl_blocked;
int arl_spmm_blocked_f32(const arl_blocked *P, const float *X, int64_t d, float alpha, float beta, const float *Z,
                         const uint8_t *zflags, float *Y, arl_stream_t stream);
int arl_spmm_csr_rscale_f32(const arl_csr *A, const float *X, int64_t d, const float *row_scale, float alpha, float beta,
                            const float *Z, float *Y, arl_stream_t stream);
int arl_spmm_blocked_rscale_f32(const arl_blocked *P, const float *X, int64_t d, const float *row_scale, float alpha,
                                float beta, const float *Z, float *Y, arl_stream_t stream);
int arl_spmm_blocked_layersum_f32(const arl_blocked *P, const float *X, int64_t d, const float *S_in, float *S, float *Y,
                                  arl_stream_t stream);
int arl_spmm_blocked_adam_f32(const arl_blocked *P, const float *X, int64_t d, float alpha, float beta, const float *Z,
                              const uint8_t *zflags, float *Pm, float *M, float *V, float lr, float beta1, float beta2,
                              float eps, int64_t step, arl_stream_t stream);
int arl_lpt_deal(int64_t n, const int32_t *weight_desc, int64_t n_bins, int64_t cap, int32_t *bin_out, int32_t *slot_out);

int64_t arl_syn_v1_pairs(int64_t n_users, int64_t n_items, double mean_deg, uint64_t seed, double sigma, int64_t deg_min, int64_t deg_max,
                         int32_t *pairs_out, int64_t capacity);
uint64_t arl_graph_digest(const int32_t *pairs, int64_t n);

typedef struct arl_tiled {
    int64_t n_sweeps, n_slots, cap, n_cb, nnz;
    int64_t n_groups;
    const int32_t *bin_rows;
    const int32_t *seg_ptr;
    const int32_t *e_col;
    const float *e_val;
    const uint16_t *e_row;
} arl_tiled;
int arl_spmm_tiled_f32(const arl_tiled *T, const float *X, int64_t d, float alpha, float beta, const float *Z,
                       const uint8_t *zflags, float *Y, arl_stream_t stream);
int arl_spmm_tiled_adam_f32(const arl_tiled *T, const float *X, int64_t d, float alpha, float beta, const float *Z,
                            const uint8_t *zflags, float *P, float *M, float *V, float lr, float beta1, float beta2,
                            float eps, int64_t step, arl_stream_t stream);

int64_t arl_bpr_l2_workspace_bytes(int64_t B);
int arl_bpr_l2_fwd_bwd_f32(const float *emb, int64_t d, int64_t item_off, const int32_t *u, const int32_t *p,
                           const int32_t *n, int64_t B, float reg, float upstream, float *loss_out, float *G,
                           void *workspace, int32_t distinct_rows, arl_stream_t stream);

int arl_bpr_l2_partial_f32(const float *emb, int64_t d, int64_t item_off, const int32_t *u, const int32_t *p,
                           const int32_t *n, int64_t B_local, int64_t B_global, float *sums_out, void *workspace,
                           arl_stream_t stream);
int arl_bpr_l2_backward_f32(const float *emb, int64_t d, int64_t item_off, const int32_t *u, const int32_t *p,
                            const int32_t *n, int64_t B_local, float reg, float upstream, const float *norms4, float *G,
                            const void *workspace, arl_stream_t stream);

int arl_adam_dense_f32(float *p, const float *g, float *m, float *v, int64_t n, float lr, float beta1,
                       float beta2, float eps, int64_t step, arl_stream_t stream);
int arl_sgd_dense_f32(float *p, const float *g, int64_t n, float lr, arl_stream_t stream);

int arl_gather_rows_f32(const float *src, const int32_t *idx, int64_t n, int64_t d, float *dst, arl_stream_t stream);
int arl_scatter_add_rows_f32(float *dst, const int32_t *idx, int64_t n, int64_t d, const float *src, float scale,
                             arl_stream_t stream);
int arl_rows_axpy_unique_f32(float *dst, const float *src, const int32_t *idx, int64_t n, int64_t d, float alpha,
                             const uint32_t *dup_bits, arl_stream_t stream);
int arl_shard_batch_prep_i32(const int32_t *u, const int32_t *p, const int32_t *n, int64_t B, int64_t u0, int64_t u1,
                             int32_t *lu, float *own, int32_t *item_rows, int32_t *rows_l, arl_stream_t stream);

int64_t arl_infonce_workspace_bytes(int64_t n, int64_t d);
int arl_infonce_fwd_bwd_f32(const float *v1, const float *v2, int64_t n, int64_t d, float tau, float upstream,
                            float *loss_out, float *dv1, float *dv2, void *workspace, arl_stream_t stream);

int arl_simgcl_perturb_f32(float *E, const float *noise, int64_t n, int64_t d, float eps, arl_stream_t stream);
int arl_simgcl_perturb_rng_f32(const float *src, float *dst, int64_t n, int64_t d, const int32_t *row_ids, float eps, uint64_t seed,
                               uint64_t stream_id, arl_stream_t stream);

int arl_ngcf_combine_f32(const float *P, const float *E, int64_t n, int64_t d, float *ST, arl_stream_t stream);
int arl_ngcf_act_f32(float *Z, float *acc, int64_t n, int64_t d, float slope, arl_stream_t stream);
int arl_ngcf_act_bwd_f32(const float *gOut, const float *Out, int64_t n, int64_t d, float slope, float *gZ, arl_stream_t stream);
int arl_ngcf_combine_bwd_f32(const float *gST, const float *P, const float *E, int64_t n, int64_t d, float *gP, float *gE,
                             arl_stream_t stream);
int arl_ngcf_dense_fwd_f32(const float *P, const float *E, const float *W, int64_t n, int64_t d, float slope, float *out, arl_stream_t stream);
int arl_ngcf_dense_dgrad_f32(const float *gOut, const float *Out, const float *P, const float *E, const float *Wt, int64_t n, int64_t d, float slope,
                             float *gZ, float *gP, float *gE, arl_stream_t stream);
int64_t arl_ngcf_wgrad_workspace_bytes(int64_t n, int64_t d);
int arl_ngcf_dense_wgrad_f32(const float *P, const float *E, const float *gZ, int64_t n, int64_t d, float *gW, void *workspace, arl_stream_t stream);

int arl_ncf_tower_fwd_f32(const float *mf, const float *mlp, const int32_t *rows, int64_t n, int64_t d, const float *W0, const float *b0,
                          const float *W1, const float *b1, const float *W2, const float *b2, float *out, float *h1, float *h2, arl_stream_t stream);
int64_t arl_ncf_tower_bwd_workspace_bytes(int64_t n, int64_t d);
int arl_ncf_tower_bwd_f32(const float *g_out, const float *out, const float *h1, const float *h2, const float *mlp, const int32_t *rows, int64_t n,
                          int64_t d, const float *W0, const float *W1, const float *W2, float *g_mlp_rows, float *g_params, void *workspace,
                          arl_stream_t stream);

int64_t arl_wrmf_l2_workspace_bytes(int64_t B);
int arl_wrmf_l2_fwd_bwd_f32(const float *emb, int64_t d, int64_t item_off, const int32_t *u, const int32_t *p, const int32_t *n, int64_t B,
                            float pos_weight, float reg, float upstream, float *loss_out, float *G, void *workspace, int32_t distinct_rows,
                            arl_stream_t stream);

int64_t arl_sfa_workspace_bytes(int64_t n_rows, int64_t d);
int arl_sfa_l1_fwd_bwd_f32(const float *X, const float *w, const float *r0, int64_t n_rows, int64_t d, int64_t numel_h,
                           float scale, int32_t accumulate, float *loss_out, float *G, void *workspace, arl_stream_t stream);
int arl_sfa_stage1_f32(const float *X, const float *w, const float *r0, int64_t n_rows, int64_t d, float *r_out, void *workspace,
                       arl_stream_t stream);
int arl_sfa_stage2_f32(const float *X, const float *w, const float *r, int64_t n_rows, int64_t d, float *as_out, void *workspace,
                       arl_stream_t stream);
int arl_sfa_stage3_f32(const float *X, const float *w, const float *r0, const float *r, const float *as, int64_t n_rows, int64_t d,
                       int64_t numel_h, float scale, int32_t accumulate, float *loss_out, float *G, void *workspace, arl_stream_t stream);

int arl_sddmm_rows_dense_f32(const float *dY, const float *X, int64_t d, const int32_t *rows, int64_t n_rows_sel,
                             int64_t col_off, int64_t n_cols, float *out, arl_stream_t stream);
int arl_sddmm_csr_f32(const int32_t *rowptr, const int32_t *col, int64_t n_rows, int64_t d, const float *dY, const float *X, float alpha,
                      float *gval, arl_stream_t stream);
int arl_tables_sum_f32(const float *const *tables, int64_t n_tables, int64_t n_elems, float alpha, float *out, arl_stream_t stream);

int64_t arl_fake_block_rows_workspace_bytes(int64_t F, int64_t I, int64_t d);
int arl_fake_block_rows_f32(const float *S, int64_t F, int64_t I, const float *X, int64_t d, const float *rscale, float alpha, float *Y,
                            void *workspace, arl_stream_t stream);
int arl_fake_block_cols_f32(const float *S, int64_t F, int64_t I, const float *Xf, int64_t d, const float *rscale, float alpha, float *Y,
                            arl_stream_t stream);
int arl_pga_update_f32(float *S, const float *grad, const float *dinv_rows, const float *dinv_cols, int64_t rows,
                       int64_t cols, arl_stream_t stream);
int64_t arl_score_mask_topk_workspace_bytes(int64_t I, int64_t d);
int64_t arl_score_mask_topk_user_workspace_bytes(int64_t U, int64_t d);
int64_t arl_score_mask_topk_stats_offset(int64_t I, int64_t d);
int arl_score_mask_topk_f32(const float *Pu, const float *Pi, int64_t U, int64_t I, int64_t d,
                            const int32_t *mask_rowptr, const int32_t *mask_col, int64_t k, int32_t *top_idx,
                            float *top_val, void *workspace, const int32_t *warm_idx, int32_t *underflow,
                            const int32_t *item_order, int32_t exit_mode, void *user_workspace, arl_stream_t stream);
int64_t arl_cw_topk_term_workspace_bytes(int64_t n_items, int64_t d, int64_t n_real, int64_t n_targets);
int arl_cw_topk_term_f32(const float *X, int64_t n_user_rows, int64_t n_items, int64_t d, int64_t n_real, const int32_t *top_idx, int64_t k,
                         const int64_t *targets, int64_t n_targets, float c, float *G, float *loss, float *w_sfa, void *workspace,
                         arl_stream_t stream);
int arl_topn_project_rows_f32(const float *M, int64_t rows, int64_t cols, int64_t n, float *out, int32_t *idx,
                              float *scratch, arl_stream_t stream);

int64_t arl_nce_allrows_workspace_bytes(int64_t nA, int64_t nV, int64_t d);
int arl_nce_allrows_lse_f32(const float *A, int64_t nA, const float *V, int64_t nV, int64_t d, float tau, float *lse,
                            void *workspace, arl_stream_t stream);
int arl_nce_allrows_grad_f32(const float *A, int64_t nA, const float *V, int64_t nV, int64_t d, float tau, float *lse, int32_t lse_given,
                             float *dA, float *dV, void *workspace, arl_stream_t stream);

int64_t arl_ssl_dropout_nce_workspace_bytes(int64_t n, int64_t d);
// ... 42 lines not shown
```

Baseline: 321,400.

## Add per-batch plan for row-subset SpMM and transposed masked pull

Introduces a batch plan built on the GPU. It dedups the batch rows, splits their adjacency into fixed-size pieces, and builds per-column transposed segments sorted for deterministic order. New kernels compute row-subset SpMM from the piece partials, and a pull-style masked SpMM covers only the nodes the batch touches. The aim is to replace full-graph or split-workspace propagation with work proportional to the batch's neighbourhood. In exchange it adds several build launches per batch, atomics, and a host sync for the overflow check in checked mode. Whether the training loop uses these paths by default is not visible.

```diff
diff --git a/arlib_amd/_lib.py b/arlib_amd/_lib.py
--- a/arlib_amd/_lib.py
+++ b/arlib_amd/_lib.py
@@ -3,7 +3,7 @@
 
 _HERE = os.path.dirname(os.path.abspath(__file__))
 LIB_PATH = os.environ.get('ARLIB_AMD_LIB') or os.path.join(_HERE, 'lib', 'libarlib_amd.so')
-ABI_VERSION = 27
+ABI_VERSION = 28
 _lib = None
 
 
@@ -28,6 +28,13 @@
     _fields_ = [('n_sweeps', C.c_int64), ('n_slots', C.c_int64), ('cap', C.c_int64), ('n_cb', C.c_int64), ('nnz', C.c_int64),
                 ('n_groups', C.c_int64), ('bin_rows', C.c_void_p), ('seg_ptr', C.c_void_p), ('e_col', C.c_void_p), ('e_val', C.c_void_p),
                 ('e_row', C.c_void_p)]
+
+
+class arl_batch_plan(C.Structure):
+    _fields_ = [('n_nodes', C.c_int64), ('cap_rows', C.c_int64), ('cap_pieces', C.c_int64), ('cap_edges', C.c_int64), ('cap_long', C.c_int64),
+                ('quantum', C.c_int64), ('node_owner', C.c_void_p), ('node_count', C.c_void_p), ('seg', C.c_void_p), ('own', C.c_void_p),
+                ('row_piece', C.c_void_p), ('pieces', C.c_void_p), ('seg_row', C.c_void_p), ('seg_val', C.c_void_p), ('long_list', C.c_void_p),
+                ('ctr', C.c_void_p), ('partial', C.c_void_p)]
 
 
 _vp, _i64, _i32, _f = C.c_void_p, C.c_int64, C.c_int32, C.c_float
@@ -56,6 +63,9 @@
     'arl_spmm_csr_flagged_f32': (C.c_int, [C.POINTER(arl_csr), _vp, _i64, _vp, _f, _f, _vp, _vp, _vp, _vp]),
     'arl_spmm_csr_rows_workspace_bytes': (_i64, [_i64, _i64, _i64]),
     'arl_spmm_csr_rows_f32': (C.c_int, [C.POINTER(arl_csr), _vp, _i64, _vp, _i64, _i64, _vp, _i64, _f, _vp, _vp, _vp, _vp]),
+    'arl_batch_plan_build': (C.c_int, [C.POINTER(arl_csr), _vp, _i64, C.POINTER(arl_batch_plan), _i32, _vp]),
+    'arl_spmm_plan_rows_f32': (C.c_int, [C.POINTER(arl_batch_plan), C.POINTER(arl_csr), _vp, _i64, _vp, _i64, _vp, _i64, _f, _vp, _vp, _vp]),
+    'arl_spmm_plan_masked_f32': (C.c_int, [C.POINTER(arl_batch_plan), _vp, _i64, _f, _f, _vp, _vp, _vp, _vp]),
     'arl_mark_rows_u8': (C.c_int, [_vp, _vp, _i64, _i32, _vp]),
     'arl_mark_rows_bits_u32': (C.c_int, [_vp, _vp, _i64, _i32, _vp]),
     'arl_zero_rows_f32': (C.c_int, [_vp, _vp, _i64, _i64, _vp]),
diff --git a/arlib_amd/csrc/arl_host.cpp b/arlib_amd/csrc/arl_host.cpp
--- a/arlib_amd/csrc/arl_host.cpp
+++ b/arlib_amd/csrc/arl_host.cpp
@@ -79,7 +79,7 @@
 
 extern "C" {
 
-int arl_abi_version(void) { return 27; }
+int arl_abi_version(void) { return 28; }
 
 int arl_mt_seed(uint32_t *mt_state, const uint32_t *key, int64_t key_len) {
     if (!mt_state || !key) return ARL_E_NULL;
diff --git a/arlib_amd/csrc/arl_kernels.hip b/arlib_amd/csrc/arl_kernels.hip
--- a/arlib_amd/csrc/arl_kernels.hip
+++ b/arlib_amd/csrc/arl_kernels.hip
@@ -273,6 +273,243 @@
     for (int s = 0; s < nsplit; ++s) a = add4(a, *reinterpret_cast<const float4 *>(partial + ((size_t)t * nsplit + s) * d + q * 4));
     const float w = row_weight ? alpha * row_weight[t] : alpha;
     *reinterpret_cast<float4 *>(out_c + (size_t)t * d + q * 4) = make_float4(w * a.x, w * a.y, w * a.z, w * a.w);
+}
+
+struct PlanDev {
+    int n_nodes, cap_pieces, cap_edges, cap_long, quantum;
+    int32_t *node_owner, *node_count;
+    int2 *seg;
+    int32_t *own;
+    int2 *row_piece;
+    int4 *pieces;
+    int32_t *seg_row;
+    float *seg_val;
+    int32_t *long_list;
+    int32_t *ctr;
+    float *partial;
+};
+constexpr int kPlanShortSeg = 32;
+constexpr int kPlanRowsBlock = 1024;
+constexpr int kPlanMaxWaves = 16384;
+
+__global__ __launch_bounds__(kBlock) void plan_owner_kernel(const int32_t *__restrict__ rows, int n, int32_t *__restrict__ node_owner) {
+    const int t = blockIdx.x * kBlock + threadIdx.x;
+    if (t < n) atomicMin(node_owner + rows[t], t);
+}
+
+__global__ __launch_bounds__(kPlanRowsBlock) void plan_rows_kernel(const int32_t *__restrict__ rowptr, const int32_t *__restrict__ rows, int n, PlanDev P) {
+    __shared__ int s_wave[kPlanRowsBlock / kWave];
+    __shared__ int s_carry;
+    __shared__ unsigned long long s_edges;
+    __shared__ int s_ok;
+    const int tid = threadIdx.x, lane = tid & 63, wv = tid >> 6;
+    if (tid == 0) { s_carry = 0; s_edges = 0ull; }
+    __syncthreads();
+    for (int base = 0; base < n; base += kPlanRowsBlock) {
+        const int t = base + tid;
+        int np = 0, deg = 0;
+        if (t < n) {
+            const int r = rows[t];
+            const int o = P.node_owner[r];
+            P.own[t] = o;
+            if (o == t) { deg = rowptr[r + 1] - rowptr[r]; np = (deg + P.quantum - 1) / P.quantum; }
+        }
+        int inc = np;
+#pragma unroll
+        for (int off = 1; off < kWave; off <<= 1) { const int v = __shfl_up(inc, off); if (lane >= off) inc += v; }
+        if (lane == kWave - 1) s_wave[wv] = inc;
+        __syncthreads();
+        int before = s_carry;
+        for (int w = 0; w < wv; ++w) before += s_wave[w];
+        if (t < n) P.row_piece[t] = make_int2(before + inc - np, np);
+        if (deg > 0) atomicAdd(&s_edges, (unsigned long long)deg);
+        __syncthreads();
+        if (tid == kPlanRowsBlock - 1) s_carry = before + inc;
+        __syncthreads();
+    }
+    if (tid == 0) {
+        const bool ok = s_carry <= P.cap_pieces && s_edges <= (unsigned long long)P.cap_edges;
+        s_ok = ok;
+        P.ctr[0] = ok ? s_carry : 0;
+        P.ctr[3] = ok ? 0 : 1;
+        P.ctr[4] = s_carry;
+        P.ctr[5] = s_edges > 0x7fffffffull ? 0x7fffffff : (int)s_edges;
+    }
+    __syncthreads();
+    for (int t = tid; t < n; t += kPlanRowsBlock) {
+        const int r = rows[t];
+        if (s_ok && P.own[t] == t) {
+            const int2 rp = P.row_piece[t];
+            const int b = rowptr[r], e = rowptr[r + 1];
+            for (int k = 0; k < rp.y; ++k) P.pieces[rp.x + k] = make_int4(r, b + k * P.quantum, min(e, b + (k + 1) * P.quantum), 0);
+        }
+        P.node_owner[r] = 0x7fffffff;
+    }
+}
+
+__global__ __launch_bounds__(kBlock) void plan_count_kernel(const int32_t *__restrict__ col, PlanDev P) {
+    const int lane = threadIdx.x & 63;
+    const int np = P.ctr[0], nw = gridDim.x * kWavesPerBlock;
+    for (int p = blockIdx.x * kWavesPerBlock + (threadIdx.x >> 6); p < np; p += nw) {
+        const int4 pc = P.pieces[p];
+        for (int e = pc.y + lane; e < pc.z; e += kWave) atomicAdd(P.node_count + col[e], 1);
+    }
+}
+
+__global__ __launch_bounds__(kBlock) void plan_alloc_kernel(PlanDev P) {
+    __shared__ int s_wave[kWavesPerBlock];
+    __shared__ int s_base;
+    const int tid = threadIdx.x, lane = tid & 63, wv = tid >> 6;
+    const int c0 = (blockIdx.x * kBlock + tid) * 4;
+    int len[4] = {0, 0, 0, 0};
+    if (c0 + 3 < P.n_nodes) {
+        const int4 v = *reinterpret_cast<const int4 *>(P.node_count + c0);
+        len[0] = v.x; len[1] = v.y; len[2] = v.z; len[3] = v.w;
+    } else {
+        for (int k = 0; k < 4; ++k) if (c0 + k < P.n_nodes) len[k] = P.node_count[c0 + k];
+    }
+    const int mine = len[0] + len[1] + len[2] + len[3];
+    int inc = mine;
+#pragma unroll
+    for (int off = 1; off < kWave; off <<= 1) { const int v = __shfl_up(inc, off); if (lane >= off) inc += v; }
+    if (lane == kWave - 1) s_wave[wv] = inc;
+    __syncthreads();
+    if (tid == 0) {
+        const int total = s_wave[0] + s_wave[1] + s_wave[2] + s_wave[3];
+        s_base = total ? atomicAdd(P.ctr + 1, total) : 0;
+    }
+    __syncthreads();
+    int at = s_base + inc - mine;
+    for (int w = 0; w < wv; ++w) at += s_wave[w];
+    for (int k = 0; k < 4; ++k) {
+        if (c0 + k >= P.n_nodes) break;
+        P.seg[c0 + k] = make_int2(at, len[k]);
+        at += len[k];
+        if (len[k] > kPlanShortSeg) {
+            const int i = atomicAdd(P.ctr + 2, 1);
+            if (i < P.cap_long) P.long_list[i] = c0 + k;
+        }
+    }
+}
+
+__global__ __launch_bounds__(kBlock) void plan_fill_kernel(const int32_t *__restrict__ col, const float *__restrict__ val, PlanDev P) {
+    const int lane = threadIdx.x & 63;
+    const int np = P.ctr[0], nw = gridDim.x * kWavesPerBlock;
+    for (int p = blockIdx.x * kWavesPerBlock + (threadIdx.x >> 6); p < np; p += nw) {
+        const int4 pc = P.pieces[p];
+        for (int e = pc.y + lane; e < pc.z; e += kWave) {
+            const int c = col[e];
+            const int slot = P.seg[c].x + atomicSub(P.node_count + c, 1) - 1;
+            if (slot >= 0 && slot < P.cap_edges) { P.seg_row[slot] = pc.x; P.seg_val[slot] = val[e]; }
+        }
+    }
+}
+
+__device__ __forceinline__ bool plan_less(int ra, float va, int rb, float vb) {
+    return ra != rb ? ra < rb : __float_as_uint(va) < __float_as_uint(vb);
+}
+
+__global__ __launch_bounds__(kBlock) void plan_sort_short_kernel(PlanDev P) {
+    const int c = blockIdx.x * kBlock + threadIdx.x;
+    if (c >= P.n_nodes) return;
+    const int2 s = P.seg[c];
+    if (s.y < 2 || s.y > kPlanShortSeg) return;
+    int32_t *r = P.seg_row + s.x;
+    float *v = P.seg_val + s.x;
+    for (int i = 1; i < s.y; ++i) {
+        const int ri = r[i];
+        const float vi = v[i];
+        int j = i - 1;
+        while (j >= 0 && plan_less(ri, vi, r[j], v[j])) { r[j + 1] = r[j]; v[j + 1] = v[j]; --j; }
+        r[j + 1] = ri; v[j + 1] = vi;
+    }
+}
+
+__global__ __launch_bounds__(kBlock) void plan_sort_long_kernel(PlanDev P, int lds_cap) {
+    extern __shared__ int32_t s_plan[];
+    int32_t *kr = s_plan;
+    float *kv = reinterpret_cast<float *>(s_plan + lds_cap);
+    const int nl = min(P.ctr[2], P.cap_long);
+    for (int i = blockIdx.x; i < nl; i += gridDim.x) {
+        const int2 s = P.seg[P.long_list[i]];
+        if (s.y > lds_cap) { if (threadIdx.x == 0) P.ctr[3] = 2; continue; }
+        for (int j = threadIdx.x; j < s.y; j += kBlock) { kr[j] = P.seg_row[s.x + j]; kv[j] = P.seg_val[s.x + j]; }
+        __syncthreads();
+        for (int j = threadIdx.x; j < s.y; j += kBlock) {
+            const int rj = kr[j];
+            const float vj = kv[j];
+            int rank = 0;
+            for (int k = 0; k < s.y; ++k) rank += (plan_less(kr[k], kv[k], rj, vj) || (k < j && kr[k] == rj && __float_as_uint(kv[k]) == __float_as_uint(vj))) ? 1 : 0;
+            P.seg_row[s.x + rank] = rj;
+            P.seg_val[s.x + rank] = vj;
+        }
+        __syncthreads();
+    }
+}
+
+template <int LPR>
+__global__ __launch_bounds__(kBlock) void plan_piece_kernel(const int32_t *__restrict__ col, const float *__restrict__ val, const float *__restrict__ X, int d, PlanDev P) {
+    const int lane = threadIdx.x & 63, q = lane % LPR;
+    const int np = P.ctr[0], nw = gridDim.x * kWavesPerBlock;
+    for (int p = blockIdx.x * kWavesPerBlock + (threadIdx.x >> 6); p < np; p += nw) {
+        const int4 pc = P.pieces[p];
+        float4 a = spmm_gather<LPR, 4>(col, val, pc.y, pc.z, X, d, lane);
+        a = group_reduce<LPR>(a);
+        if (lane < LPR && q * 4 < d) *reinterpret_cast<float4 *>(P.partial + (size_t)p * d + q * 4) = a;
+    }
+}
+
+template <int LPR>
+__global__ __launch_bounds__(kBlock) void plan_finish_kernel(PlanDev P, int n, int d, const int32_t *__restrict__ rows, LayerPtrs L, float alpha,
+                                                              float *__restrict__ out_c, const float *__restrict__ row_weight) {
+    constexpr int G = kWave / LPR;
+    const int lane = threadIdx.x & 63, g = lane / LPR, q = lane % LPR;
+    const int t = blockIdx.x * kWavesPerBlock + (threadIdx.x >> 6);
+    if (t >= n || P.ctr[3] != 0) return;
+    const int2 rp = P.row_piece[P.own[t]];
+    const bool qact = q * 4 < d;
+    float4 a = make_float4(0.f, 0.f, 0.f, 0.f);
+    if (qact) {
+        const float *pp = P.partial + (size_t)rp.x * d + q * 4;
+        int s = g;
+        for (; s + 3 * G < rp.y; s += 4 * G) {
+            const float4 x0 = *reinterpret_cast<const float4 *>(pp + (size_t)s * d), x1 = *reinterpret_cast<const float4 *>(pp + (size_t)(s + G) * d);
+            const float4 x2 = *reinterpret_cast<const float4 *>(pp + (size_t)(s + 2 * G) * d), x3 = *reinterpret_cast<const float4 *>(pp + (size_t)(s + 3 * G) * d);
+            a = add4(add4(add4(add4(a, x0), x1), x2), x3);
+        }
+        for (; s < rp.y; s += G) a = add4(a, *reinterpret_cast<const float4 *>(pp + (size_t)s * d));
+    }
+    a = group_reduce<LPR>(a);
+    if (lane >= LPR || !qact) return;
+    const int r = rows[t];
+    float4 l = make_float4(0.f, 0.f, 0.f, 0.f);
+    for (int k = 0; k < L.n; ++k) l = add4(l, *reinterpret_cast<const float4 *>(L.p[k] + (size_t)r * d + q * 4));
+    a = add4(l, a);
+    const float w = row_weight ? alpha * row_weight[t] : alpha;
+    *reinterpret_cast<float4 *>(out_c + (size_t)t * d + q * 4) = make_float4(w * a.x, w * a.y, w * a.z, w * a.w);
+}
+
+template <int LPR>
+__global__ __launch_bounds__(kBlock) void plan_pull_kernel(PlanDev P, const float *__restrict__ X, int d, Epi ep) {
+    constexpr int G = kWave / LPR;
+    const int lane = threadIdx.x & 63, g = lane / LPR, q = lane % LPR;
+    const long long c = ((long long)blockIdx.x * kWavesPerBlock + (threadIdx.x >> 6)) * G + g;
+    if (c >= P.n_nodes || q * 4 >= d || P.ctr[3] != 0) return;
+    const int2 s = P.seg[c];
+    const int32_t *sr = P.seg_row + s.x;
+    const float *sv = P.seg_val + s.x;
+    const float *xq = X + q * 4;
+    float4 acc = make_float4(0.f, 0.f, 0.f, 0.f);
+    int i = 0;
+    for (; i + 3 < s.y; i += 4) {
+        const int r0 = sr[i], r1 = sr[i + 1], r2 = sr[i + 2], r3 = sr[i + 3];
+        const float v0 = sv[i], v1 = sv[i + 1], v2 = sv[i + 2], v3 = sv[i + 3];
+        const float4 x0 = *reinterpret_cast<const float4 *>(xq + (size_t)r0 * d), x1 = *reinterpret_cast<const float4 *>(xq + (size_t)r1 * d);
+        const float4 x2 = *reinterpret_cast<const float4 *>(xq + (size_t)r2 * d), x3 = *reinterpret_cast<const float4 *>(xq + (size_t)r3 * d);
+        fma4(acc, v0, x0); fma4(acc, v1, x1); fma4(acc, v2, x2); fma4(acc, v3, x3);
+    }
+    for (; i < s.y; ++i) fma4(acc, sv[i], *reinterpret_cast<const float4 *>(xq + (size_t)sr[i] * d));
+    spmm_epilogue<EPI_AXPBY>(ep, (int)c, d, q, acc);
 }
 
 __global__ __launch_bounds__(kBlock) void tables_sum_kernel(LayerPtrs L, long long n4, float alpha, float4 *__restrict__ out) {
@@ -4212,6 +4449,124 @@
     else if (d <= 128) ARL_SUBSET_CASE(32);
     else ARL_SUBSET_CASE(64);
 #undef ARL_SUBSET_CASE
+    return ARL_OK;
+}
+
+static int plan_dev(const arl_batch_plan *P, PlanDev &D) {
+    if (!P || !P->node_owner || !P->node_count || !P->seg || !P->own || !P->row_piece || !P->pieces || !P->seg_row || !P->seg_val || !P->long_list ||
+        !P->ctr || !P->partial) return ARL_E_NULL;
+    if (P->n_nodes <= 0 || P->n_nodes > 0x7fffffffll || P->cap_rows <= 0 || P->cap_rows > ARL_PLAN_MAX_ROWS || P->cap_pieces <= 0 || P->cap_pieces > 0x7fffffffll ||
+        P->cap_edges <= 0 || P->cap_edges > 0x7fffffffll || P->quantum < 64 || P->quantum > 65536) return ARL_E_RANGE;
+    if (P->cap_long < P->cap_edges / (kPlanShortSeg + 1) + 1 || P->cap_long > 0x7fffffffll) return ARL_E_ARG;
+    if (((uintptr_t)P->node_count | (uintptr_t)P->pieces | (uintptr_t)P->partial) & 15 || ((uintptr_t)P->seg | (uintptr_t)P->row_piece) & 7) return ARL_E_ARG;
+    D.n_nodes = (int)P->n_nodes; D.cap_pieces = (int)P->cap_pieces; D.cap_edges = (int)P->cap_edges; D.cap_long = (int)P->cap_long; D.quantum = (int)P->quantum;
+    D.node_owner = P->node_owner; D.node_count = P->node_count; D.seg = reinterpret_cast<int2 *>(P->seg); D.own = P->own;
+    D.row_piece = reinterpret_cast<int2 *>(P->row_piece); D.pieces = reinterpret_cast<int4 *>(P->pieces); D.seg_row = P->seg_row; D.seg_val = P->seg_val;
+    D.long_list = P->long_list; D.ctr = P->ctr; D.partial = P->partial;
+    return ARL_OK;
+}
+
+static unsigned plan_piece_grid(const PlanDev &D) {
+    const int waves = D.cap_pieces < kPlanMaxWaves ? D.cap_pieces : kPlanMaxWaves;
+    return (unsigned)((waves + kWavesPerBlock - 1) / kWavesPerBlock);
+}
+
+int arl_batch_plan_build(const arl_csr *A, const int32_t *rows, int64_t n, const arl_batch_plan *P, int32_t stages, arl_stream_t stream) {
+    PlanDev D;
+    const int rc = plan_dev(P, D);
+    if (rc) return rc;
+    if (!A || !rows || !A->rowptr || (A->nnz > 0 && (!A->col || !A->val))) return ARL_E_NULL;
+    if (A->n_rows != P->n_nodes || n < 0 || n > P->cap_rows || !(stages & 3)) return ARL_E_ARG;
+    hipStream_t st = (hipStream_t)stream;
+    hipError_t e;
+    if (stages & 1) {
+        if ((e = hipMemsetAsync(D.ctr, 0, 8 * sizeof(int32_t), st)) != hipSuccess) return (int)e;
+        if (n > 0) {
+            hipLaunchKernelGGL(plan_owner_kernel, dim3((unsigned)((n + kBlock - 1) / kBlock)), dim3(kBlock), 0, st, rows, (int)n, D.node_owner);
+            ARL_LAUNCH_CHECK();
+            hipLaunchKernelGGL(plan_rows_kernel, dim3(1), dim3(kPlanRowsBlock), 0, st, A->rowptr, rows, (int)n, D);
+            ARL_LAUNCH_CHECK();
+        }
+    }
+    if (stages & 2) {
+        if ((e = hipMemsetAsync(D.ctr + 1, 0, 2 * sizeof(int32_t), st)) != hipSuccess) return (int)e;
+        const unsigned gp = plan_piece_grid(D);
+        hipLaunchKernelGGL(plan_count_kernel, dim3(gp), dim3(kBlock), 0, st, A->col, D);
+        ARL_LAUNCH_CHECK();
+        hipLaunchKernelGGL(plan_alloc_kernel, dim3((unsigned)((D.n_nodes + 4 * kBlock - 1) / (4 * kBlock))), dim3(kBlock), 0, st, D);
+        ARL_LAUNCH_CHECK();
+        hipLaunchKernelGGL(plan_fill_kernel, dim3(gp), dim3(kBlock), 0, st, A->col, A->val, D);
+        ARL_LAUNCH_CHECK();
+        hipLaunchKernelGGL(plan_sort_short_kernel, dim3((unsigned)((D.n_nodes + kBlock - 1) / kBlock)), dim3(kBlock), 0, st, D);
+        ARL_LAUNCH_CHECK();
+        const int lds_cap = n > 64 ? (int)n : 64;
+        const size_t shm = (size_t)lds_cap * 8;
+        if (shm > 64 * 1024 && (e = hipFuncSetAttribute((const void *)plan_sort_long_kernel, hipFuncAttributeMaxDynamicSharedMemorySize, (int)shm)) != hipSuccess)
+            return (int)e;
+        const unsigned gl = (unsigned)(D.cap_long < 1024 ? D.cap_long : 1024);
+        hipLaunchKernelGGL(plan_sort_long_kernel, dim3(gl), dim3(kBlock), shm, st, D, lds_cap);
+        ARL_LAUNCH_CHECK();
+    }
+    return ARL_OK;
+}
+
+int arl_spmm_plan_rows_f32(const arl_batch_plan *P, const arl_csr *A, const float *X, int64_t d, const int32_t *rows, int64_t n_rows_sel,
+                           const float *const *layers, int64_t n_layers, float alpha, const float *row_weight, float *out_c, arl_stream_t stream) {
+    PlanDev D;
+    const int rc = plan_dev(P, D);
+    if (rc) return rc;
+    if (!A || !X || !rows || !out_c || (A->nnz > 0 && (!A->col || !A->val))) return ARL_E_NULL;
+    if (n_layers < 0 || n_layers > 8 || (n_layers > 0 && !layers)) return ARL_E_ARG;
+    if (d <= 0 || d > 256 || (d & 3)) return ARL_E_DIM;
+    if (A->n_rows != P->n_nodes || n_rows_sel < 0 || n_rows_sel > P->cap_rows) return ARL_E_ARG;
+    if (n_rows_sel == 0) return ARL_OK;
+    hipStream_t st = (hipStream_t)stream;
+    LayerPtrs LP = {};
+    LP.n = (int)n_layers;
+    for (int k = 0; k < LP.n; ++k) { if (!layers[k]) return ARL_E_NULL; LP.p[k] = layers[k]; }
+    const int di = (int)d, n = (int)n_rows_sel;
+    const unsigned gp = plan_piece_grid(D), gf = (unsigned)((n + kWavesPerBlock - 1) / kWavesPerBlock);
+#define ARL_PLAN_ROWS_CASE(LPRV)                                                                                                \
+    do {                                                                                                                        \
+        hipLaunchKernelGGL((plan_piece_kernel<LPRV>), dim3(gp), dim3(kBlock), 0, st, A->col, A->val, X, di, D);                 \
+        ARL_LAUNCH_CHECK();                                                                                                     \
+        hipLaunchKernelGGL((plan_finish_kernel<LPRV>), dim3(gf), dim3(kBlock), 0, st, D, n, di, rows, LP, alpha, out_c, row_weight); \
+        ARL_LAUNCH_CHECK();                                                                                                     \
+    } while (0)
+    if (d <= 16) ARL_PLAN_ROWS_CASE(4);
+    else if (d <= 32) ARL_PLAN_ROWS_CASE(8);
+    else if (d <= 64) ARL_PLAN_ROWS_CASE(16);
+    else if (d <= 128) ARL_PLAN_ROWS_CASE(32);
+    else ARL_PLAN_ROWS_CASE(64);
+#undef ARL_PLAN_ROWS_CASE
+    return ARL_OK;
+}
+
+int arl_spmm_plan_masked_f32(const arl_batch_plan *P, const float *X, int64_t d, float alpha, float beta, const float *Z, const uint8_t *zflags,
+                             float *Y, arl_stream_t stream) {
+    PlanDev D;
+    const int rc = plan_dev(P, D);
+    if (rc) return rc;
+    if (!X || !Y) return ARL_E_NULL;
+    if (beta != 0.f && !Z) return ARL_E_NULL;
+    if (Y == X) return ARL_E_ARG;
+    if (d <= 0 || d > 256 || (d & 3)) return ARL_E_DIM;
+    Epi ep = {};
+    ep.alpha = alpha; ep.beta = beta; ep.Z = (beta != 0.f) ? Z : nullptr; ep.zflags = zflags; ep.Y = Y;
+    hipStream_t st = (hipStream_t)stream;
+    const int di = (int)d;
+#define ARL_PLAN_PULL_CASE(LPRV)                                                                                                \
+    do {                                                                                                                        \
+        const long long per = (long long)kWavesPerBlock * (kWave / LPRV);                                                       \
+        hipLaunchKernelGGL((plan_pull_kernel<LPRV>), dim3((unsigned)((D.n_nodes + per - 1) / per)), dim3(kBlock), 0, st, D, X, di, ep); \
+        ARL_LAUNCH_CHECK();                                                                                                     \
+    } while (0)
+    if (d <= 16) ARL_PLAN_PULL_CASE(4);
+    else if (d <= 32) ARL_PLAN_PULL_CASE(8);
+    else if (d <= 64) ARL_PLAN_PULL_CASE(16);
+    else if (d <= 128) ARL_PLAN_PULL_CASE(32);
+    else ARL_PLAN_PULL_CASE(64);
+#undef ARL_PLAN_PULL_CASE
     return ARL_OK;
 }
 
diff --git a/arlib_amd/engine.py b/arlib_amd/engine.py
--- a/arlib_amd/engine.py
+++ b/arlib_amd/engine.py
@@ -23,7 +23,7 @@
 
 class PropagationEngine:
     def __init__(self, graph, n_users, n_items, emb_size, n_layers, reg, lr, device, skip_layer0=False,
-                 optimizer='adam', betas=(0.9, 0.999), eps=1e-8, table=None, schedule='auto'):
+                 optimizer='adam', betas=(0.9, 0.999), eps=1e-8, table=None, schedule='auto', batch_plan='auto', plan_edges=None):
         self.A = graph
         self.U, self.I, self.d, self.L = int(n_users), int(n_items), int(emb_size), int(n_layers)
         self.N = self.U + self.I
@@ -43,6 +43,11 @@
             raise ValueError('skip_layer0 needs n_layers >= 1')
         if schedule not in ('auto', 'csr', 'blocked'):
             raise ValueError("schedule must be 'auto', 'csr' or 'blocked'")
+        if batch_plan not in ('auto', 'on', 'off'):
+            raise ValueError("batch_plan must be 'auto', 'on' or 'off'")
+        self.batch_plan, self.plan_edges = batch_plan, plan_edges
+        self._plan = self._deg_prefix = None
+        self._plan_live = False
         if schedule != 'csr':
             ops.auto_blocked(graph, emb_size, split=self.U, force=(schedule == 'blocked'))
         if graph is not None and graph.nnz >= ops.BLOCKED_MIN_NNZ:
@@ -142,7 +147,7 @@
         self._begin_sparse(self._sparse_B)
         self._set_rows(rows, g_rows.contiguous())
         acc, bits = self._masked_hops(A, self.hops)
-        out = ops.spmm_flagged(A, acc, bits, s, s, self.G, self.flags)
+        out = self._flagged(A, acc, bits, s, s, self.G, self.flags)
         self._clear_rows(rows)
         return out
 
@@ -172,7 +177,33 @@
         layers = [self.E0]
         for k in range(self.L - 1):
             layers.append(ops.spmm(graph, layers[-1], out=hops[k]))
+        plan = self._plan_for(graph, rows)
+        if plan is not None:
+            res = ops.spmm_rows_plan(plan, layers[-1], rows, layers, 1.0 / (self.L + 1), out=out, build=True)
+            if res is not None:
+                return res
         return ops.spmm_rows(graph, layers[-1], rows, layers, 1.0 / (self.L + 1), nsplit=self.nsplit, out=out, workspace=workspace, check_range=False)
+
+    def _plan_for(self, graph, rows):
+        n = rows.numel()
+        if self.batch_plan == 'off' or graph is not self.A or graph.n_cols != graph.n_rows or n == 0 or n > ops.PLAN_MAX_ROWS:
+            return None
+        if self.batch_plan == 'auto' and graph.nnz < ops.BLOCKED_MIN_NNZ:
+            return None
+        p = self._plan
+        if p is None or p.cap_rows < n:
+            if self._deg_prefix is None:
+                deg = torch.sort((graph.rowptr[1:] - graph.rowptr[:-1]).long(), descending=True)[0]
+                self._deg_prefix = torch.cumsum(deg, 0).cpu()
+            bound = max(int(self._deg_prefix[min(n, graph.n_rows) - 1]), 1)
+            cap = min(bound, ops.PLAN_MAX_EDGES if self.plan_edges is None else int(self.plan_edges))
+            p = self._plan = ops.BatchPlan(graph, n, cap, self.d, max_edges=bound)
+        return p
+
+    def _flagged(self, graph, X, bits, alpha, beta, Z, zflags, out=None):
+        if bits is not None and self._plan_live and graph is self.A:
+            return ops.spmm_flagged_plan(self._plan, X, alpha, beta, Z, zflags, out=out)
+        return ops.spmm_flagged(graph, X, bits, alpha, beta, Z, zflags, out=out)
 
     def _bpr_compact(self, out_c, B):
         self.Gc.zero_()
@@ -180,6 +211,7 @@
 
     def _set_rows(self, rows, grad):
         ops.batch_rows_set_(self.G, self.flags, self.bits, rows, grad, 1.0, check_range=False, dup_bits=self.dup_bits)
+        self._plan_live = self._plan is not None and self._plan.rows is rows
 
     def _mark_rows(self, rows):
         ops.mark_rows_(self.flags, rows, 1, check_range=False)
@@ -187,11 +219,14 @@
 
     def _clear_rows(self, rows):
         ops.batch_rows_clear_(self.G, self.flags, self.bits, rows, check_range=False, dup_bits=self.dup_bits)
+        if self._plan is not None:
+            self._plan.invalidate()
+        self._plan_live = False
 
     def _masked_hops(self, graph, bufs, src=None, after_hop=None):
         acc, bits = self.G if src is None else src, self.bits
         for k in range(self.L - 1):
-            acc = ops.spmm_flagged(graph, acc, bits, 1.0, 1.0, self.G, self.flags, out=bufs[k % len(bufs)])
+            acc = self._flagged(graph, acc, bits, 1.0, 1.0, self.G, self.flags, out=bufs[k % len(bufs)])
             bits = None
             if after_hop is not None:
                 after_hop(self.L - 1 - k, acc)
@@ -230,7 +265,7 @@
         self.t += 1
         acc, bits = self._masked_hops(A, self.hops)
         if L == 1:
-            ops.spmm_flagged(A, acc, bits, s, s, self.G, self.flags, out=self.hops[0])
+            self._flagged(A, acc, bits, s, s, self.G, self.flags, out=self.hops[0])
             ops.adam_dense(self.E0, self.hops[0], self.m, self.v, self.lr, self.t, self.betas, self.eps)
         else:
             ops.spmm_adam(A, acc, s, s, self.G, self.E0, self.m, self.v, self.lr, self.t, self.betas, self.eps, zflags=self.flags)
@@ -460,7 +495,7 @@
         def backward_into(graph, sel, grad_c, accumulate):
             self._set_rows(sel, grad_c)
             acc, bits = self._masked_hops(graph, self._sgl_hops)
-            tmp = ops.spmm_flagged(graph, acc, bits, s, s, self.G, self.flags, out=self._sgl_hops[0] if L == 1 else self.hops[0])
+            tmp = self._flagged(graph, acc, bits, s, s, self.G, self.flags, out=self._sgl_hops[0] if L == 1 else self.hops[0])
             if accumulate:
                 self._sgl_acc.add_(tmp)
             else:
diff --git a/arlib_amd/ops.py b/arlib_amd/ops.py
--- a/arlib_amd/ops.py
+++ b/arlib_amd/ops.py
@@ -688,6 +688,146 @@
     return out
 
 
+PLAN_QUANTUM = 256
+PLAN_MAX_ROWS = 16384
+PLAN_MAX_EDGES = 1 << 27
+
+
+class BatchPlan:
+
+    def __init__(self, A, cap_rows, cap_edges, d, max_edges=None, grow_to=None, quantum=PLAN_QUANTUM):
+        if A.n_cols != A.n_rows:
+            raise ValueError('BatchPlan: square (symmetric) adjacency only')
+        if not (0 < cap_rows <= PLAN_MAX_ROWS):
+            raise ValueError('BatchPlan: 1 .. %d listed rows' % PLAN_MAX_ROWS)
+        _check_width(d, 'BatchPlan')
+        self.A, self.d, self.quantum, self.cap_rows = A, int(d), int(quantum), int(cap_rows)
+        self.max_edges = None if max_edges is None else int(max_edges)
+        self.grow_to = max(int(cap_edges), int(grow_to if grow_to is not None else (max_edges if max_edges is not None else A.nnz)))
+        dev, N = A.device, A.n_rows
+        self.node_owner = torch.full((N,), 0x7fffffff, dtype=torch.int32, device=dev)
+        self.node_count = torch.zeros(N, dtype=torch.int32, device=dev)
+        self.seg = torch.zeros(N, 2, dtype=torch.int32, device=dev)
+        self.own = torch.zeros(self.cap_rows, dtype=torch.int32, device=dev)
+        self.row_piece = torch.zeros(self.cap_rows, 2, dtype=torch.int32, device=dev)
+        self.ctr = torch.zeros(8, dtype=torch.int32, device=dev)
+        self.stats = {'builds': 0, 'checked': 0, 'overflows': 0, 'grown': 0, 'failed': 0}
+        self.rows = None
+        self.segments = False
+        self._size(max(int(cap_edges), 1))
+
+    def _size(self, cap_edges):
+        dev = self.A.device
+        self.cap_edges = int(cap_edges)
+        self.cap_pieces = self.cap_rows + self.cap_edges // self.quantum + 1
+        self.cap_long = self.cap_edges // 33 + 1
+        self.pieces = torch.zeros(self.cap_pieces, 4, dtype=torch.int32, device=dev)
+        self.seg_row = torch.zeros(self.cap_edges, dtype=torch.int32, device=dev)
+        self.seg_val = torch.zeros(self.cap_edges, dtype=torch.float32, device=dev)
+        self.long_list = torch.zeros(self.cap_long, dtype=torch.int32, device=dev)
+        self.partial = torch.empty(self.cap_pieces * self.d, dtype=torch.float32, device=dev)
+        s = _lib.arl_batch_plan()
+        s.n_nodes, s.cap_rows, s.cap_pieces, s.cap_edges, s.cap_long, s.quantum = self.A.n_rows, self.cap_rows, self.cap_pieces, self.cap_edges, self.cap_long, self.quantum
+        for nm in ('node_owner', 'node_count', 'seg', 'own', 'row_piece', 'pieces', 'seg_row', 'seg_val', 'long_list', 'ctr', 'partial'):
+            setattr(s, nm, getattr(self, nm).data_ptr())
+        self._s = s
+
+    @property
+    def checked(self):
+        return self.max_edges is None or self.cap_edges < self.max_edges
+
+    def _launch(self, rows, stages):
+        check(_lib.lib().arl_batch_plan_build(C.byref(self.A._struct(self.d)), _ptr(rows), rows.numel(), C.byref(self._s), stages, _stream()), 'arl_batch_plan_build')
+
+    def build(self, rows, check_range=True):
+        _dev(rows, torch.int32, 'rows', 1)
+        n = rows.numel()
+        if n > self.cap_rows:
+            raise ValueError('BatchPlan.build: %d rows, room for %d' % (n, self.cap_rows))
+        if check_range and n and (int(rows.min()) < 0 or int(rows.max()) >= self.A.n_rows):
+            raise IndexError('BatchPlan.build: row index out of range')
+        self.rows, self.segments = None, False
+        self._launch(rows, 1)
+        self.stats['builds'] += 1
+        if self.checked:
+            self.stats['checked'] += 1
+            c = self.ctr.cpu()
+            if int(c[3]):
+                self.stats['overflows'] += 1
+                need = int(c[5])
+                if need > self.grow_to:
+                    self.stats['failed'] += 1
+                    return False
+                self._size(min(self.grow_to, max(need, need + need // 4)))
+                self.stats['grown'] += 1
+                self._launch(rows, 1)
+                if int(self.ctr.cpu()[3]):
+                    self.stats['failed'] += 1
+                    return False
+        self.rows = rows
+        return True
+
+    def build_segments(self):
+        if self.rows is None:
+            raise _lib.ArlError('BatchPlan.build_segments: no valid plan')
+        if not self.segments:
+            self._launch(self.rows, 2)
+            self.segments = True
+
+    def invalidate(self):
+        self.rows, self.segments = None, False
+
+
+def spmm_rows_plan(plan, X, rows, layers=(), alpha=1.0, out=None, row_weight=None, build=False, check_range=False):
+    A = plan.A
+    d = _check_xy(A, X, 'X', A.n_cols)
+    if d != plan.d or (not build and plan.rows is not rows):
+        raise _lib.ArlError('spmm_rows_plan: the plan was not built for these rows / this width')
+    n = rows.numel()
+    if len(layers) > 8:
+        raise ValueError('spmm_rows_plan: at most 8 layer tables')
+    for t in layers:
+        if _check_xy(A, t, 'layer') != d:
+            raise ValueError('spmm_rows_plan: layer table shape mismatch')
+    if out is None:
+        out = torch.empty(n, d, dtype=torch.float32, device=X.device)
+    _dev(out, torch.float32, 'out', 2)
+    if out.shape != (n, d):
+        raise ValueError('spmm_rows_plan: out must be [len(rows), d]')
+    if row_weight is not None and (_dev(row_weight, torch.float32, 'row_weight', 1).numel() != n):
+        raise ValueError('spmm_rows_plan: row_weight must have one entry per listed row')
+    arr = (C.c_void_p * max(len(layers), 1))(*[t.data_ptr() for t in layers])
+    tok = EVENT_HOOK.begin('rows') if EVENT_HOOK is not None else None
+    ok = plan.build(rows, check_range=check_range) if build else True
+    if ok:
+        check(_lib.lib().arl_spmm_plan_rows_f32(C.byref(plan._s), C.byref(A._struct(d)), _ptr(X), d, _ptr(rows), n, C.cast(arr, C.c_void_p), len(layers), alpha,
+                                                _ptr(row_weight), _ptr(out), _stream()), 'arl_spmm_plan_rows_f32')
+    if tok is not None:
+        EVENT_HOOK.end(tok)
+    return out if ok else None
+
+
+def spmm_flagged_plan(plan, X, alpha=1.0, beta=0.0, Z=None, zflags=None, out=None):
+    A = plan.A
+    d = _check_xy(A, X, 'X', A.n_cols)
+    if plan.rows is None or d != plan.d:
+        raise _lib.ArlError('spmm_flagged_plan: no valid plan for this width')
+    Y = torch.empty(A.n_rows, d, dtype=torch.float32, device=X.device) if out is None else out
+    if _check_xy(A, Y, 'out') != d or Y.data_ptr() == X.data_ptr():
+        raise ValueError('spmm_flagged_plan: out must be [n_rows, d] and must not alias X')
+    if beta != 0.0 and (Z is None or _check_xy(A, Z, 'Z') != d):
+        raise ValueError('spmm_flagged_plan: Z [n_rows, d] required when beta != 0')
+    if zflags is not None:
+        _check_flags(zflags, A.n_rows, 'zflags')
+    tok = EVENT_HOOK.begin('masked') if EVENT_HOOK is not None else None
+    plan.build_segments()
+    check(_lib.lib().arl_spmm_plan_masked_f32(C.byref(plan._s), _ptr(X), d, alpha, beta, _ptr(Z) if beta != 0.0 else None, _ptr(zflags), _ptr(Y), _stream()),
+          'arl_spmm_plan_masked_f32')
+    if tok is not None:
+        EVENT_HOOK.end(tok)
+    return Y
+
+
 def mark_rows_(flags, idx, value, check_range=True):
     _dev(flags, torch.uint8, 'flags', 1); _dev(idx, torch.int32, 'idx', 1)
     if check_range and idx.numel() and (int(idx.min()) < 0 or int(idx.max()) >= flags.numel()):
diff --git a/include/arlib_amd.h b/include/arlib_amd.h
--- a/include/arlib_amd.h
+++ b/include/arlib_amd.h
@@ -64,6 +64,28 @@
 int arl_spmm_csr_rows_f32(const arl_csr *A, const float *X, int64_t d, const int32_t *rows, int64_t n_rows_sel,
                           int64_t nsplit, const float *const *layers, int64_t n_layers, float alpha, const float *row_weight,
                           float *out_c, void *workspace, arl_stream_t stream);
+
+#define ARL_PLAN_MAX_ROWS 16384
+typedef struct arl_batch_plan {
+    int64_t n_nodes, cap_rows, cap_pieces, cap_edges, cap_long, quantum;
+    int32_t *node_owner;
+    int32_t *node_count;
+    int32_t *seg;
+    int32_t *own;
+    int32_t *row_piece;
+    int32_t *pieces;
+    int32_t *seg_row;
+    float *seg_val;
+    int32_t *long_list;
+    int32_t *ctr;
+    float *partial;
+} arl_batch_plan;
+int arl_batch_plan_build(const arl_csr *A, const int32_t *rows, int64_t n, const arl_batch_plan *P, int32_t stages, arl_stream_t stream);
+int arl_spmm_plan_rows_f32(const arl_batch_plan *P, const arl_csr *A, const float *X, int64_t d, const int32_t *rows, int64_t n_rows_sel,
+                           const float *const *layers, int64_t n_layers, float alpha, const float *row_weight, float *out_c,
+                           arl_stream_t stream);
+int arl_spmm_plan_masked_f32(const arl_batch_plan *P, const float *X, int64_t d, float alpha, float beta, const float *Z,
+                             const uint8_t *zflags, float *Y, arl_stream_t stream);
 int arl_mark_rows_u8(uint8_t *flags, const int32_t *idx, int64_t n, int32_t value, arl_stream_t stream);
 int arl_mark_rows_bits_u32(uint32_t *bits, const int32_t *idx, int64_t n, int32_t set, arl_stream_t stream);
 int arl_zero_rows_f32(float *dst, const int32_t *idx, int64_t n, int64_t d, arl_stream_t stream);
```

Result: slower. 311,400 (-3.1%).
